# fluggo/Canvas

Hardware: AMD Instinct MI355X
Metric: Mpixels/s through 4K f16 RGBA colour-matrix+alpha-over chain; % HBM roofline (higher is better)
Workload: dtype f32

## Files before the change

### canvas_amd/_lib.py

```python
import ctypes as C
import os

from .abi import (box2i, fir_filter, rational, rgba_frame_f16, rgba_frame_f32, v2f, video_frame_source_funcs,
                  video_source)

_HERE = os.path.dirname(os.path.abspath(__file__))
LIB_PATH = os.path.join(_HERE, "libcanvas_hip.so")

CHAIN_MAX_LAYERS = 8
DISPLAY_RGBA8, DISPLAY_ARGB32_PREMUL = 0, 1
FIR_PATH_AUTO, FIR_PATH_PASSES, FIR_PATH_TILED, FIR_PATH_TABLES, FIR_PATH_HV, FIR_PATH_ONE_COLUMN, FIR_PATH_TWO_COLUMNS, FIR_PATH_STRIPS, FIR_PATH_TILES = 0, 1, 2, 4, 16, 32, 64, 128, 256
FIR_KERNEL_NONE, FIR_KERNEL_WINDOW, FIR_KERNEL_HALVE, _FIR_KERNEL_RETIRED_3, FIR_KERNEL_VH, FIR_KERNEL_TILED, _FIR_KERNEL_RETIRED_6, FIR_KERNEL_TWO_PASS, FIR_KERNEL_PASS, FIR_KERNEL_HV, FIR_KERNEL_WINDOW_PAIR, FIR_KERNEL_HALVE_PAIR, FIR_KERNEL_TILE_VH, FIR_KERNEL_UNSHARP = range(14)
ARITH_SEPARATE, ARITH_CONTRACTED = 0, 1
LUT_NONE, LUT_REC709_TO_LINEAR_SCENE, LUT_REC709_TO_LINEAR_DISPLAY, LUT_LINEAR_TO_REC709, LUT_LINEAR_TO_SRGB = -1, 0, 1, 2, 3
KEY_SHOW_MATTE = 1
MATTE_SHOW, MATTE_MAX_CHOKE, MATTE_MAX_TAPS = 1, 16, 25
TRANSFORM_NEAREST, TRANSFORM_BILINEAR, TRANSFORM_MAX_COORD = 0, 1, 1 << 23
MAX_COORD, RESAMPLE_MAX_COORD = 1 << 30, 1 << 23
YCC_PROGRESSIVE, YCC_REC709 = 1, 2


class rgba_f32(C.Structure):
    _fields_ = [("r", C.c_float), ("g", C.c_float), ("b", C.c_float), ("a", C.c_float)]


class rgba_frame_dev(C.Structure):
    _fields_ = [("data", C.c_void_p), ("format", C.c_int), ("full_window", box2i), ("current_window", box2i),
                ("stream", C.c_void_p)]


class chain_job(C.Structure):
    _fields_ = [("out", C.POINTER(rgba_frame_f16)), ("layers", C.POINTER(rgba_frame_f16) * CHAIN_MAX_LAYERS),
                ("nlayers", C.c_int)]


class chroma_key(C.Structure):
    _fields_ = [("key", C.c_float * 3), ("tolerance", C.c_float), ("softness", C.c_float), ("spill", C.c_float),
                ("spill_range", C.c_float), ("flags", C.c_int)]


class matte_params(C.Structure):
    _fields_ = [("black", C.c_float), ("white", C.c_float), ("choke", C.c_int), ("ntaps", C.c_int), ("taps", C.POINTER(C.c_float)),
                ("flags", C.c_int)]


def matte(choke=0, feather=None, black=0.0, white=1.0, show_matte=False):
    taps = [float(t) for t in feather] if feather is not None else []
    array = (C.c_float * len(taps))(*taps) if taps else None
    m = matte_params(black, white, int(choke), len(taps), C.cast(array, C.POINTER(C.c_float)) if taps else None, MATTE_SHOW if show_matte else 0)
    m._taps = array
    return m


class transform_params(C.Structure):
    _fields_ = [("m", C.c_float * 6), ("filter", C.c_int), ("flags", C.c_int)]


def transform(m=(1.0, 0.0, 0.0, 0.0, 1.0, 0.0), filter=TRANSFORM_BILINEAR):
    return transform_params((C.c_float * 6)(*[float(v) for v in m]), int(filter), 0)


class coded_image(C.Structure):
    _fields_ = [("data", C.c_void_p * 4), ("stride", C.c_int * 4), ("line_count", C.c_int * 4), ("free_func", C.c_void_p)]


P = C.POINTER
rgba_frame_f16_t = rgba_frame_f16
rgba_frame_f32_t = rgba_frame_f32
_u16p, _f32p, _vp = P(C.c_uint16), P(C.c_float), C.c_void_p
_F16, _F32 = P(rgba_frame_f16), P(rgba_frame_f32)

SIGNATURES = {
    "init_half": (None, []),
    "get_frame_time": (C.c_int64, [P(rational), C.c_int]),
    "get_time_frame": (C.c_int, [P(rational), C.c_int64]),
    "gettime": (C.c_int64, []),
    "video_get_frame_f16": (None, [P(video_source), C.c_int, _F16]),
    "video_get_frame_f32": (None, [P(video_source), C.c_int, _F32]),
    "video_get_frame_f16_gl": (None, [P(video_source), C.c_int, _F16]),
    "video_get_frame_f32_gl": (None, [P(video_source), C.c_int, _F32]),
    "video_get_frame_dev": (None, [P(video_source), C.c_int, P(rgba_frame_dev)]),
    "video_copy_frame_f16": (None, [_F16, _F16]),
    "video_copy_frame_alpha_f32": (None, [_F32, _F32, C.c_float]),
    "video_attenuate_f32": (None, [_F32, C.c_float]),
    "cvs_pulldown23_frames": (C.c_int, [C.c_int, C.c_int, P(C.c_int), P(C.c_int)]),
    "cvs_weave_fields_f16_dev": (C.c_int, [_F16, _F16, _vp]),
    "cvs_field_to_frame_f16_dev": (C.c_int, [_F16, _F16, C.c_int, _vp]),
    "cvs_soften_fields_f16_dev": (C.c_int, [_F16, _F16, _vp]),
    "cvs_interlace_fields_f16_dev": (C.c_int, [_F16, _F16, _F16, _vp]),
    "cvs_pulldown23_add_frames": (C.c_int, [C.c_int, C.c_int, P(C.c_int), P(C.c_int)]),
    "video_mix_cross_f32": (None, [_F32, _F32, _F32, C.c_float]),
    "video_mix_cross_f32_pull": (None, [_F32, P(video_source), C.c_int, P(video_source), C.c_int, C.c_float]),
    "video_mix_over_f32": (None, [_F32, _F32, C.c_float]),
    "video_scale_bilinear_f32": (None, [_F32, v2f, _F32, v2f, v2f]),
    "video_scale_bilinear_f32_pull": (None, [_F32, v2f, P(video_source), C.c_int, P(box2i), v2f, v2f]),
    "video_transfer_rec709_to_linear_scene": (None, [_u16p, _u16p, C.c_size_t]),
    "video_transfer_rec709_to_linear_display": (None, [_u16p, _u16p, C.c_size_t]),
    "video_transfer_linear_to_rec709": (None, [_u16p, _u16p, C.c_size_t]),
    "video_transfer_linear_to_sRGB": (None, [_u16p, _u16p, C.c_size_t]),
    "video_get_gamma45_ramp": (P(C.c_uint8), []),
    "video_color_rgb_to_xyz_sdtv": (None, [_F16]),
    "video_color_xyz_to_srgb": (None, [_F16]),
    "filter_createTriangle": (None, [C.c_float, C.c_float, P(fir_filter)]),
    "filter_createLanczos": (None, [C.c_float, C.c_int, C.c_float, P(fir_filter)]),
    "filter_free": (None, [P(fir_filter)]),
    "video_filter_gain_offset_f16": (None, [_F16, _F16, C.c_float, C.c_float]),
    "video_fill_solid_f16": (None, [_F16, P(box2i), P(rgba_f32)]),
    "video_fill_solid_f32": (None, [_F32, P(box2i), P(rgba_f32)]),
    "workspace_create": (_vp, []),
    "workspace_get_length": (C.c_int, [_vp]),
    "workspace_add_item": (_vp, [_vp, _vp, C.c_int64, C.c_int64, C.c_int64, C.c_int64, _vp]),
    "workspace_get_item": (_vp, [_vp, C.c_int]),
    "workspace_remove_item": (None, [_vp]),
    "workspace_as_video_source": (None, [_vp, P(video_source)]),
    "workspace_free": (None, [_vp]),
    "workspace_get_item_pos": (None, [_vp, P(C.c_int64), P(C.c_int64), P(C.c_int64)]),
    "workspace_get_item_offset": (C.c_int64, [_vp]),
    "workspace_set_item_offset": (None, [_vp, C.c_int64]),
    "workspace_get_item_source": (_vp, [_vp]),
    "workspace_set_item_source": (None, [_vp, _vp]),
    "workspace_get_item_tag": (_vp, [_vp]),
    "workspace_set_item_tag": (None, [_vp, _vp]),
    "workspace_update_item": (None, [_vp, P(C.c_int64), P(C.c_int64), P(C.c_int64), P(C.c_int64), P(_vp), P(_vp)]),
    "cvs_set_arithmetic": (C.c_int, [C.c_int]),
    "cvs_get_arithmetic": (C.c_int, []),
    "cvs_init": (C.c_int, [C.c_int]),
    "cvs_device_count": (C.c_int, []),
    "cvs_current_device": (C.c_int, []),
    "cvs_context_open": (C.c_int, [C.c_int]),
    "cvs_context_count": (C.c_int, []),
    "cvs_context_device": (C.c_int, [C.c_int]),
    "cvs_set_context": (C.c_int, [C.c_int]),
    "cvs_current_context": (C.c_int, []),
    "cvs_frame_owner": (C.c_int, [C.c_int64, C.c_int]),
    "cvs_last_error": (C.c_char_p, []),
    "cvs_clear_last_error": (None, []),
    "cvs_set_log_handler": (None, [C.c_void_p, C.c_void_p]),
    "cvs_device_name": (C.c_char_p, []),
    "cvs_compute_units": (C.c_int, []),
    "cvs_malloc": (_vp, [C.c_size_t]),
    "cvs_free": (None, [_vp]),
    "cvs_graph_begin": (C.c_int, [_vp]),
    "cvs_graph_end": (_vp, [_vp]),
    "cvs_graph_launch": (C.c_int, [_vp, _vp]),
    "cvs_graph_destroy": (None, [_vp]),
    "cvs_mem_info": (C.c_int, [P(C.c_size_t), P(C.c_size_t)]),
    "cvs_pool_malloc": (_vp, [C.c_size_t, _vp]),
    "cvs_pool_free": (None, [_vp, _vp]),
    "cvs_pool_trim": (None, []),
    "cvs_thread_release": (None, []),
    "cvs_memcpy_h2d": (C.c_int, [_vp, _vp, C.c_size_t, _vp]),
    "cvs_memcpy_d2h": (C.c_int, [_vp, _vp, C.c_size_t, _vp]),
    "cvs_memcpy_d2d": (C.c_int, [_vp, _vp, C.c_size_t, _vp]),
    "cvs_memset": (C.c_int, [_vp, C.c_int, C.c_size_t, _vp]),
    "cvs_stream_create": (_vp, []),
    "cvs_stream_destroy": (None, [_vp]),
    "cvs_stream_sync": (C.c_int, [_vp]),
    "cvs_event_create": (_vp, []),
    "cvs_event_destroy": (None, [_vp]),
    "cvs_event_record": (C.c_int, [_vp, _vp]),
    "cvs_event_sync": (C.c_int, [_vp]),
    "cvs_event_elapsed_ms": (C.c_float, [_vp, _vp]),
    "cvs_lut_device": (_vp, [C.c_int]),
    "cvs_lut_host": (_u16p, [C.c_int]),
    "cvs_lut_install": (C.c_int, [C.c_int, _u16p]),
    "cvs_half_to_float_dev": (C.c_int, [_vp, _vp, C.c_size_t, _vp]),
    "cvs_float_to_half_dev": (C.c_int, [_vp, _vp, C.c_size_t, _vp]),
    "cvs_half_to_float_fast_dev": (C.c_int, [_vp, _vp, C.c_size_t, _vp]),
    "cvs_float_to_half_fast_dev": (C.c_int, [_vp, _vp, C.c_size_t, _vp]),
    "cvs_half_lookup_dev": (C.c_int, [_vp, _vp, _vp, C.c_size_t, _vp]),
    "cvs_frame_f16_to_f32_dev": (C.c_int, [_F32, _F16, _vp]),
    "cvs_frame_f32_to_f16_dev": (C.c_int, [_F16, _F32, _vp]),
    "cvs_copy_frame_f16_dev": (C.c_int, [_F16, _F16, _vp]),
    "cvs_copy_frame_alpha_f32_dev": (C.c_int, [_F32, _F32, C.c_float, _vp]),
    "cvs_mix_cross_f32_dev": (C.c_int, [_F32, _F32, _F32, C.c_float, _vp]),
    "cvs_mix_over_f32_dev": (C.c_int, [_F32, _F32, C.c_float, _vp]),
    "cvs_color_matrix_f16_dev": (C.c_int, [_F16, _f32p, C.c_int, C.c_int, _vp]),
    "cvs_color_matrix_f16_to_dev": (C.c_int, [_F16, _F16, _f32p, C.c_int, C.c_int, _vp]),
    "cvs_gain_offset_f16_dev": (C.c_int, [_F16, _F16, C.c_float, C.c_float, _vp]),
    "cvs_fill_solid_f16_dev": (C.c_int, [_F16, P(box2i), P(rgba_f32), _vp]),
    "cvs_fill_solid_f32_dev": (C.c_int, [_F32, P(box2i), P(rgba_f32), _vp]),
    "cvs_scale_bilinear_f16_dev": (C.c_int, [_F16, v2f, _F16, v2f, v2f, _vp]),
    "cvs_scale_bilinear_f32_dev": (C.c_int, [_F32, v2f, _F32, v2f, v2f, _vp]),
    "cvs_fir_blur_f32_dev": (C.c_int, [_F32, _F32, _f32p, C.c_int, _vp]),
    "coded_image_alloc": (P(coded_image), [P(C.c_int), P(C.c_int), C.c_int]),
    "coded_image_alloc0": (P(coded_image), [P(C.c_int), P(C.c_int), C.c_int]),
    "video_reconstruct_dv": (None, [_F16, P(coded_image)]),
    "video_subsample_dv": (P(coded_image), [_F16]),
    "cvs_reconstruct_dv_dev": (C.c_int, [_F16, P(coded_image), _vp]),
    "cvs_subsample_dv_dev": (C.c_int, [P(coded_image), _F16, C.c_int, _vp]),
    "video_subsample_mpeg2": (P(coded_image), [_F16]),
    "cvs_subsample_mpeg2_dev": (C.c_int, [P(coded_image), _F16, C.c_int, C.c_int, _vp]),
    "video_reconstruct_mpeg2": (None, [_F16, P(coded_image)]),
    "cvs_reconstruct_mpeg2_dev": (C.c_int, [_F16, P(coded_image), C.c_int, C.c_int, C.c_int, _vp]),
    "cvs_frame_to_bytes_dev": (C.c_int, [_vp, _F16, C.c_int, C.c_int, _vp]),
    "video_frame_to_bytes": (C.c_int, [_vp, _F16, C.c_int, C.c_int]),
    "cvs_frame_to_rgba8_intent_dev": (C.c_int, [_vp, _F16, C.c_int, C.c_float, _vp]),
    "video_frame_to_rgba8_intent": (C.c_int, [_vp, _F16, C.c_int, C.c_float]),
    "cvs_fir_blur_f16_dev": (C.c_int, [_F16, _F16, _f32p, C.c_int, _vp]),
    "cvs_unsharp_mask_f32_dev": (C.c_int, [_F32, _F32, _f32p, C.c_int, C.c_float, C.c_float, _vp]),
    "cvs_unsharp_mask_f16_dev": (C.c_int, [_F16, _F16, _f32p, C.c_int, C.c_float, C.c_float, _vp]),
    "cvs_chroma_key_f32_dev": (C.c_int, [_F32, _F32, P(chroma_key), _vp]),
    "cvs_chroma_key_f16_dev": (C.c_int, [_F16, _F16, P(chroma_key), _vp]),
    "cvs_matte_refine_f32_dev": (C.c_int, [_F32, _F32, P(matte_params), _vp]),
    "cvs_matte_refine_f16_dev": (C.c_int, [_F16, _F16, P(matte_params), _vp]),
    "cvs_transform_f32_dev": (C.c_int, [_F32, _F32, P(transform_params), _vp]),
    "cvs_transform_f16_dev": (C.c_int, [_F16, _F16, P(transform_params), _vp]),
    "cvs_transform_from_parts": (C.c_int, [P(C.c_double), P(C.c_double), C.c_double, P(C.c_double), _f32p]),
    "cvs_transform_target_window": (C.c_int, [P(transform_params), P(box2i), P(box2i), P(box2i)]),
    "cvs_transform_source_window": (C.c_int, [P(transform_params), P(box2i), P(box2i)]),
    "cvs_blur_over_f16_dev": (C.c_int, [_F16, _F16, _f32p, C.c_int, P(_F16), C.c_int, _vp]),
    "cvs_resample_lanczos_f32_dev": (C.c_int, [_F32, _F32, C.c_float, C.c_float, C.c_int, _vp]),
    "cvs_resample_lanczos_f16_dev": (C.c_int, [_F16, _F16, C.c_float, C.c_float, C.c_int, _vp]),
    "cvs_blur_lanczos_f16_dev": (C.c_int, [_F16, _F16, _f32p, C.c_int, C.c_float, C.c_float, C.c_int, _vp]),
    "cvs_blur_over_f16_batch_dev": (C.c_int, [P(_F16), P(_F16), _f32p, C.c_int, P(_F16), C.c_int, C.c_int, _vp]),
    "cvs_scale_bilinear_f16_batch_dev": (C.c_int, [P(_F16), v2f, P(_F16), v2f, v2f, C.c_int, _vp]),
    "cvs_scale_bilinear_f32_batch_dev": (C.c_int, [P(_F32), v2f, P(_F32), v2f, v2f, C.c_int, _vp]),
    "cvs_blur_lanczos_f16_batch_dev": (C.c_int, [P(_F16), P(_F16), C.c_int, _f32p, C.c_int, C.c_float, C.c_float, C.c_int, _vp]),
    "cvs_fir_path_override": (None, [C.c_int]),
    "cvs_chain_color_over_f16_dev": (C.c_int, [P(chain_job), C.c_int, _f32p, C.c_int, C.c_int, _vp]),
    "cvs_chain_last_was_fused": (C.c_int, []),
    "cvs_scale_last_was_fused": (C.c_int, []),
    "cvs_fir_last_kernel": (C.c_int, []),
    "cvs_fir_fell_through_count": (C.c_int, []),
    "cvs_chain_last_launch_count": (C.c_int, []),
    "cvs_mix_cross_f16_dev": (C.c_int, [_F16, _F16, _F16, C.c_float, _vp]),
}

HALF_POINTER_GLOBALS = {
    "half_convert_to_float": C.CFUNCTYPE(None, _f32p, _u16p, C.c_int),
    "half_convert_from_float": C.CFUNCTYPE(None, _u16p, _f32p, C.c_int),
    "half_convert_to_float_fast": C.CFUNCTYPE(None, _f32p, _u16p, C.c_int),
    "half_convert_from_float_fast": C.CFUNCTYPE(None, _u16p, _f32p, C.c_int),
    "half_lookup": C.CFUNCTYPE(None, _u16p, _u16p, _u16p, C.c_int),
}

_lib = None


class LibraryMissing(RuntimeError):
    pass


def load():
    global _lib
    if _lib is not None:
        return _lib
    if not os.path.exists(LIB_PATH):
        raise LibraryMissing(
            "%s not found: build it with `python -c 'import __graft_entry__ as g; g.build()'` "
            "(or make -C canvas_amd/csrc).  There is no CPU fallback." % LIB_PATH)
    lib = C.CDLL(LIB_PATH, mode=C.RTLD_GLOBAL)
    for name, (res, args) in SIGNATURES.items():
        fn = getattr(lib, name)
        fn.restype, fn.argtypes = res, args
    _lib = lib
    return lib


def half_pointer(name):
    lib = load()
    addr = C.c_void_p.in_dll(lib, name).value
    return HALF_POINTER_GLOBALS[name](addr) if addr else None


def last_error():
    return load().cvs_last_error().decode()


def check(rc, what="call"):
    if rc != 0:
        raise RuntimeError("%s failed (%d): %s" % (what, rc, last_error()))
```

### canvas_amd/csrc/host/scale.c

```c
#define _GNU_SOURCE
#include "internal.h"
#include <limits.h>
#include <math.h>
#include <stdatomic.h>

static _Atomic int g_fir_path = CVS_FIR_PATH_AUTO;

static _Thread_local int t_scale_fused;
CVS_EXPORT int cvs_scale_last_was_fused(void) { return t_scale_fused; }
static _Thread_local int t_fir_kernel;
CVS_EXPORT int cvs_fir_last_kernel(void) { return t_fir_kernel; }
static _Thread_local int t_fell_through;
CVS_EXPORT int cvs_fir_fell_through_count(void) { return t_fell_through; }
static void fir_launch_fell_through(const char *kernel, int rc) {
    (void)hipGetLastError();
    t_fell_through++;
    cvs_log_warning("%s did not launch (%s): falling back to the next FIR kernel", kernel, hipGetErrorString((hipError_t)rc));
}
CVS_EXPORT void cvs_fir_path_override(int mode) { atomic_store(&g_fir_path, mode & (CVS_FIR_PATH_PASSES | CVS_FIR_PATH_TILED | CVS_FIR_PATH_TABLES | CVS_FIR_PATH_HV | CVS_FIR_PATH_ONE_COLUMN | CVS_FIR_PATH_TWO_COLUMNS | CVS_FIR_PATH_STRIPS | CVS_FIR_PATH_TILES)); }

typedef struct { void *data; box2i full, cur; int half; } any_frame;

static size_t any_bytes(const any_frame *f) { return cvs_box_pixels(&f->full) * (f->half ? sizeof(rgba_f16) : sizeof(rgba_f32)); }

typedef struct { void *frame, *data; box2i *full, *cur; } frame_ref;

static frame_ref frame_of(const void *f, int half) {
    frame_ref r = { (void *)f, NULL, NULL, NULL };
    if (f && half) { rgba_frame_f16 *h = r.frame; r.data = h->data; r.full = &h->full_window; r.cur = &h->current_window; }
    else if (f)    { rgba_frame_f32 *g = r.frame; r.data = g->data; r.full = &g->full_window; r.cur = &g->current_window; }
    return r;
}

static frame_ref frame_at(const void *frames, int i, int half) {
    return frame_of(half ? (const void *)((const rgba_frame_f16 *const *)frames)[i] : (const void *)((const rgba_frame_f32 *const *)frames)[i], half);
}

static any_frame any_of(const frame_ref *f, int half) {
    const any_frame a = { f->data, *f->full, *f->cur, half };
    return a;
}

static bool entry_refused(void *target, const void *source, int half, const char *what, frame_ref *t, frame_ref *src, int lim) {
    *t = frame_of(target, half);
    *src = frame_of(source, half);
    if (cvs_enter() != 0) { box2i_set_empty(t->cur); return true; }
    if (!cvs_box_contains(src->full, src->cur)) {
        cvs_set_error("%s: the input's current_window lies outside its buffer", what);
        box2i_set_empty(t->cur);
        return true;
    }
    if (cvs_coords_refused(what, "source", src->full, src->cur, lim) || cvs_coords_refused(what, "target", t->full, NULL, lim)) {
        box2i_set_empty(t->cur);
        return true;
    }
    return false;
}

static void batch_empty_from(const void *targets, int from, int count, int half) {
    for (int i = from; i < count; i++) box2i_set_empty(frame_at(targets, i, half).cur);
}

static bool batch_refused(const void *targets, const void *sources, int count, int half, const char *what, int lim) {
    if (!targets || !sources) { cvs_set_error("%s: bad arguments", what); return true; }
    for (int i = 0; i < count; i++)
        if (!frame_at(targets, i, half).frame || !frame_at(sources, i, half).frame) {
            cvs_set_error("%s: frame %d of %d is a null pointer", what, i, count);
            return true;
        }
    for (int i = 0; i < count; i++) {
        const frame_ref src = frame_at(sources, i, half);
        if (!cvs_box_contains(src.full, src.cur)) {
            cvs_set_error("%s: the input's current_window lies outside its buffer (frame %d)", what, i);
            batch_empty_from(targets, 0, count, half);
            return true;
        }
        if (cvs_coords_refused(what, "a source", src.full, src.cur, lim) || cvs_coords_refused(what, "a target", frame_at(targets, i, half).full, NULL, lim)) {
            batch_empty_from(targets, 0, count, half);
            return true;
        }
    }
    if (cvs_enter() != 0) { batch_empty_from(targets, 0, count, half); return true; }
    return false;
}

static bool same_box(const box2i *a, const box2i *b) { return memcmp(a, b, sizeof *a) == 0; }

static bool batch_group(cvk_frame_batch *b, const void *targets, const void *sources, int half, int first, int n, size_t tbytes, size_t sbytes,
                        const rgba_frame_f16 *const *overlays, int noverlays) {
    const void *in[CVK_FRAME_BATCH * (1 + CVK_BLUR_MAX_OVER)];
    int nin = 0;
    memset(b, 0, sizeof *b);
    b->n = n;
    for (int i = 0; i < n; i++) {
        b->target[i] = frame_at(targets, first + i, half).data;
        in[nin++] = b->source[i] = frame_at(sources, first + i, half).data;
        for (int l = 0; l < noverlays; l++) in[nin++] = b->over[i][l] = overlays[(size_t)(first + i) * noverlays + l]->data;
    }
    if (n < 2) return false;
    for (int i = 0; i < n; i++) {
        const char *o = b->target[i];
        for (int j = 0; j < nin; j++) { const char *q = in[j]; if (q && o < q + sbytes && q < o + tbytes) return false; }
        for (int j = 0; j < i; j++) { const char *q = b->target[j]; if (o < q + tbytes && q < o + tbytes) return false; }
    }
    return true;
}

static int gather_pass(const any_frame *t, const any_frame *src, const cvk_fir_axis *tab, int axis, int t0, int t1, int lo, int hi, hipStream_t s) {
    if (t1 < t0 || hi < lo) return 0;
    cvk_fir_params fp;
    memset(&fp, 0, sizeof fp);
    fp.target = cvs_view(t->data, &t->full);
    fp.source = cvs_view(src->data, &src->full);
    fp.axis = axis;
    fp.t0 = t0; fp.t1 = t1; fp.lo = lo; fp.hi = hi;
    fp.ntaps = tab->ntaps; fp.tap_src = tab->src; fp.taps = tab->taps; fp.stride = tab->stride;
    fp.in_half = src->half; fp.out_half = t->half;
    return CVK(cvk_fir_gather)(&fp, s);
}

static cvk_fir2d_params fir2d_params(const any_frame *t, const any_frame *src, int tx0, int ty0, int tx1, int ty1,
                                     const cvs_fir_table *h, const cvs_fir_table *v) {
    cvk_fir2d_params fp;
    memset(&fp, 0, sizeof fp);
    fp.target = cvs_view(t->data, &t->full);
    fp.source = cvs_view(src->data, &src->full);
    fp.in_half = src->half; fp.out_half = t->half;
    fp.tx0 = tx0; fp.ty0 = ty0; fp.tx1 = tx1; fp.ty1 = ty1;
    fp.h = h->axis; fp.v = v->axis;
    fp.max_sw = h->max_foot > 0 ? h->max_foot : 1;
    return fp;
}


static int triangle_pass(any_frame *target, float tmin, const any_frame *source, float smin, float factor, int axis, hipStream_t s) {
    const box2i srect = source->cur, trect = target->full;
    const int lo = axis ? (srect.min.y > trect.min.y ? srect.min.y : trect.min.y) : (srect.min.x > trect.min.x ? srect.min.x : trect.min.x);
    const int hi = axis ? (srect.max.y < trect.max.y ? srect.max.y : trect.max.y) : (srect.max.x < trect.max.x ? srect.max.x : trect.max.x);
    const int s0 = axis ? srect.min.x : srect.min.y, s1 = axis ? srect.max.x : srect.max.y;
    const int t0 = axis ? trect.min.x : trect.min.y, t1 = axis ? trect.max.x : trect.max.y;

    cvs_fir_table table;
    int rc = cvs_fir_table_triangle(tmin, smin, factor, s0, s1, t0, t1, axis == 0 || lo <= hi, &table);
    if (rc != 0) return rc;
    const int used_lo = table.used_lo, used_hi = table.used_hi;
    {
        const int o0 = axis ? trect.min.y : trect.min.x, o1 = axis ? trect.max.y : trect.max.x;
        const bool covers = used_hi >= used_lo && hi >= lo && used_lo == t0 && used_hi == t1 && lo == o0 && hi == o1;
        if (!covers && any_bytes(target)) {
            hipError_t e_ = hipMemsetAsync(target->data, 0, any_bytes(target), s);
            if (e_ != hipSuccess) { cvs_fir_table_release(&table, s); cvs_set_error("zero fill: %s", hipGetErrorString(e_)); return -1; }
        }
    }
    if (used_hi >= used_lo && hi >= lo) {
        const size_t first = (size_t)(used_lo - t0);
        cvk_fir_axis from = table.axis;
        from.ntaps += first; from.src += first * (size_t)from.stride; from.taps += first * (size_t)from.stride;
        rc = gather_pass(target, source, &from, axis, used_lo, used_hi, lo, hi, s);
        if (rc == 0) t_fir_kernel = CVS_FIR_KERNEL_PASS;
    }
    cvs_fir_table_release(&table, s);
    if (rc != 0) { cvs_set_error("FIR gather launch failed: %s", hipGetErrorString((hipError_t)rc)); return rc; }
    if (axis) box2i_set(&target->cur, used_lo, lo, used_hi, hi);
    else      box2i_set(&target->cur, lo, used_lo, hi, used_hi);
    return 0;
}

static int triangle_fused_vh(any_frame *target, v2f tp, const any_frame *source, v2f sp, v2f fac, const box2i *mid_full,
                             const cvk_frame_batch *batch, hipStream_t s) {
    const box2i *tf = &target->full, *sc = &source->cur;
    const int lo1 = sc->min.x > mid_full->min.x ? sc->min.x : mid_full->min.x, hi1 = sc->max.x < mid_full->max.x ? sc->max.x : mid_full->max.x;
    cvs_fir_table tv, th = { .pin = -1 };
    if (hi1 < lo1) return 1;
    if (cvs_fir_table_triangle(tp.y, sp.y, fac.y, sc->min.y, sc->max.y, mid_full->min.y, mid_full->max.y, true, &tv) != 0) return -1;
    const int vlo = tv.used_lo, vhi = tv.used_hi;
    int rc = 1;
    if (vhi >= vlo) {
        const int lo2 = vlo > tf->min.y ? vlo : tf->min.y, hi2 = vhi < tf->max.y ? vhi : tf->max.y;
        if (hi2 >= lo2 && cvs_fir_table_triangle(tp.x, sp.x, fac.x, lo1, hi1, tf->min.x, tf->max.x, true, &th) == 0) {
            const int hlo = th.used_lo, hhi = th.used_hi;
            cvk_fir2d_params fp = fir2d_params(target, source, tf->min.x, mid_full->min.y, tf->max.x, hi2, &th, &tv);
            const int pinned = atomic_load(&g_fir_path);
            const bool tiles = hhi >= hlo && !(pinned & CVS_FIR_PATH_STRIPS) &&
                               ((pinned & CVS_FIR_PATH_TILES) ? CVK(cvk_fir_tvh_supported)(&fp)
                                : batch && target->half ? false : CVK(cvk_fir_tvh_preferred)(&fp));
            bool alike = true;
            for (int i = 0; batch && i < batch->n; i++) alike = alike && !((((uintptr_t)batch->target[i]) ^ (uintptr_t)target->data) & 15u);
            if (batch && !(alike && hhi >= hlo && (tiles || CVK(cvk_fir_vh_supported)(&fp)))) rc = 2;
            else if (hhi >= hlo && (tiles || CVK(cvk_fir_vh_supported)(&fp))) {
                const bool covers = lo2 == tf->min.y && hi2 == tf->max.y;
                hipError_t e = hipSuccess;
                if (batch) {
                    fp.nframes = batch->n;
                    for (int i = 0; i < batch->n; i++) {
                        fp.frame_source[i] = batch->source[i]; fp.frame_target[i] = batch->target[i];
                        if (!covers && any_bytes(target) && e == hipSuccess) e = hipMemsetAsync(batch->target[i], 0, any_bytes(target), s);
                    }
                } else if (!covers && any_bytes(target)) e = hipMemsetAsync(target->data, 0, any_bytes(target), s);
                int krc = e != hipSuccess ? (int)e : tiles ? CVK(cvk_fir_tvh)(&fp, lo2 - fp.ty0, s) : CVK(cvk_fir_vh)(&fp, lo2 - fp.ty0, cvs_cus(), s);
                if (krc == 0) { box2i_set(&target->cur, hlo, lo2, hhi, hi2); t_fir_kernel = tiles ? CVS_FIR_KERNEL_TILE_VH : CVS_FIR_KERNEL_VH; rc = 0; }
                else { fir_launch_fell_through(tiles ? "k_fir_tile_vh" : "k_fir_vh", krc); rc = 1; }
            }
        }
    }
    cvs_fir_table_release(&tv, s); cvs_fir_table_release(&th, s);
    return rc;
}

static int triangle_fused_hv(any_frame *target, v2f tp, const any_frame *source, v2f sp, v2f fac, const box2i *mid_full, hipStream_t s) {
    const box2i *tf = &target->full, *sc = &source->cur;
    const int lo1 = sc->min.y > mid_full->min.y ? sc->min.y : mid_full->min.y, hi1 = sc->max.y < mid_full->max.y ? sc->max.y : mid_full->max.y;
    cvs_fir_table th, tv = { .pin = -1 };
    if (hi1 < lo1) return 1;
    if (cvs_arith() != CVS_ARITH_SEPARATE) return 1;
    if (cvs_fir_table_triangle(tp.x, sp.x, fac.x, sc->min.x, sc->max.x, mid_full->min.x, mid_full->max.x, true, &th) != 0) return -1;
    const int hlo = th.used_lo, hhi = th.used_hi;
    int rc = 1;
    if (hhi >= hlo) {
        const int lo2 = hlo > tf->min.x ? hlo : tf->min.x, hi2 = hhi < tf->max.x ? hhi : tf->max.x;
        if (hi2 >= lo2 && cvs_fir_table_triangle(tp.y, sp.y, fac.y, lo1, hi1, tf->min.y, tf->max.y, true, &tv) == 0) {
            const int vlo = tv.used_lo, vhi = tv.used_hi;
            cvk_fir2d_params fp = fir2d_params(target, source, mid_full->min.x, tf->min.y, hi2, tf->max.y, &th, &tv);
            if (vhi >= vlo && cvk_fir_hv_supported(&fp)) {
                const bool covers = fp.tx0 == tf->min.x && hi2 == tf->max.x;
                hipError_t e = covers || !any_bytes(target) ? hipSuccess : hipMemsetAsync(target->data, 0, any_bytes(target), s);
                int krc = e != hipSuccess ? (int)e : cvk_fir_hv(&fp, cvs_cus(), s);
                if (krc == 0) { box2i_set(&target->cur, lo2, vlo, hi2, vhi); t_fir_kernel = CVS_FIR_KERNEL_HV; rc = 0; }
                else { fir_launch_fell_through("k_fir_hv", krc); rc = 1; }
            }
        }
    }
    cvs_fir_table_release(&tv, s); cvs_fir_table_release(&th, s);
    return rc;
}

static int scale_core(any_frame *target, v2f tp, const any_frame *source, v2f sp, v2f fac, const cvk_frame_batch *batch, hipStream_t s) {
    t_scale_fused = 0;
    t_fir_kernel = CVS_FIR_KERNEL_NONE;
    if (batch && ((fac.x == 1.0f && tp.x == sp.x) || (fac.y == 1.0f && tp.y == sp.y) || fac.x < fac.y ||
                  (atomic_load(&g_fir_path) & (CVS_FIR_PATH_PASSES | CVS_FIR_PATH_TILED)))) return 2;
    if (fac.x == 1.0f && tp.x == sp.x) return triangle_pass(target, tp.y, source, sp.y, fac.y, 0, s);
    if (fac.y == 1.0f && tp.y == sp.y) return triangle_pass(target, tp.x, source, sp.x, fac.x, 1, s);

    any_frame mid;
    memset(&mid, 0, sizeof mid);
    const box2i *tf = &target->full, *sc = &source->cur;
    const bool x_first = fac.x < fac.y;
    const int fl = cvs_arith() == CVS_ARITH_CONTRACTED;
    if (x_first)
        box2i_set(&mid.full, (int)madd_as(fl, -(tp.x - tf->min.x), fac.x, sp.x), sc->min.y,
                  (int)madd_as(fl, tf->max.x - tp.x, fac.x, sp.x), sc->max.y);
    else
        box2i_set(&mid.full, sc->min.x, (int)madd_as(fl, -(tp.y - tf->min.y), fac.y, sp.y),
                  sc->max.x, (int)madd_as(fl, tf->max.y - tp.y, fac.y, sp.y));
    box2i_intersect(&mid.full, &mid.full, tf);
    mid.cur = mid.full;
    if (!(atomic_load(&g_fir_path) & (CVS_FIR_PATH_PASSES | CVS_FIR_PATH_TILED))) {
        int rc = x_first ? triangle_fused_hv(target, tp, source, sp, fac, &mid.full, s) : triangle_fused_vh(target, tp, source, sp, fac, &mid.full, batch, s);
        if (rc == 0) t_scale_fused = 1;
        if (rc <= 0) return rc;
        if (batch) return 2;
    }
    size_t n = cvs_box_pixels(&mid.full);
    mid.data = cvs_pool_malloc(sizeof(rgba_f32) * (n ? n : 1), s);
    if (!mid.data) return -1;
    int rc;
    if (x_first) { rc = triangle_pass(&mid, tp.x, source, sp.x, fac.x, 1, s); if (rc == 0) rc = triangle_pass(target, tp.y, &mid, sp.y, fac.y, 0, s); }
    else         { rc = triangle_pass(&mid, tp.y, source, sp.y, fac.y, 0, s); if (rc == 0) rc = triangle_pass(target, tp.x, &mid, sp.x, fac.x, 1, s); }
    cvs_pool_free(mid.data, s);
    return rc;
}

static int scale_frame(void *target, v2f tp, const void *source, v2f sp, v2f fac, int half, cvs_stream_t stream, const char *what) {
    frame_ref t, src;
    if (entry_refused(target, source, half, what, &t, &src, CVS_RESAMPLE_MAX_COORD)) return -1;
    if (cvs_point_refused(what, "the target point", tp, CVS_RESAMPLE_MAX_COORD) || cvs_point_refused(what, "the source point", sp, CVS_RESAMPLE_MAX_COORD)) {
        box2i_set_empty(t.cur);
        return -1;
    }
    hipStream_t s = cvs_pick_stream(stream);
    if (fac.x == 1.0f && tp.x == sp.x && fac.y == 1.0f && tp.y == sp.y)
        return half ? cvs_copy_frame_f16_dev(target, source, s) : cvs_copy_frame_alpha_f32_dev(target, source, 1.0f, s);
    any_frame tf = any_of(&t, half);
    const any_frame sf = any_of(&src, half);
    int rc = scale_core(&tf, tp, &sf, sp, fac, NULL, s);
    *t.cur = tf.cur;
    if (rc != 0) box2i_set_empty(t.cur);
    return rc;
}

CVS_EXPORT int cvs_scale_bilinear_f32_dev(rgba_frame_f32 *target, v2f tp, const rgba_frame_f32 *source, v2f sp, v2f fac, cvs_stream_t stream) {
    return scale_frame(target, tp, source, sp, fac, 0, stream, "cvs_scale_bilinear_f32_dev");
}

CVS_EXPORT int cvs_scale_bilinear_f16_dev(rgba_frame_f16 *target, v2f tp, const rgba_frame_f16 *source, v2f sp, v2f fac, cvs_stream_t stream) {
    return scale_frame(target, tp, source, sp, fac, 1, stream, "cvs_scale_bilinear_f16_dev");
}

static int scale_batch_frames(const void *targets, v2f tp, const void *sources, v2f sp, v2f fac, int count, int half,
                              cvs_stream_t stream, const char *what) {
    if (count <= 0) return 0;
    if (batch_refused(targets, sources, count, half, what, CVS_RESAMPLE_MAX_COORD)) return -1;
    if (cvs_point_refused(what, "the target point", tp, CVS_RESAMPLE_MAX_COORD) || cvs_point_refused(what, "the source point", sp, CVS_RESAMPLE_MAX_COORD)) {
        batch_empty_from(targets, 0, count, half);
        return -1;
    }
    hipStream_t s = cvs_pick_stream(stream);
    const size_t px = half ? sizeof(rgba_f16) : sizeof(rgba_f32);
    int rc = 0, done = 0;
    for (int base = 0; count > 1 && rc == 0 && done == base && base < count; base += 64) {
        const int end = count - base < 64 ? count : base + 64;
        const frame_ref t0 = frame_at(targets, base, half), s0 = frame_at(sources, base, half);
        bool uniform = end - base > 1 && !box2i_is_empty(s0.cur) && !box2i_is_empty(t0.full) &&
                       !(fac.x == 1.0f && tp.x == sp.x && fac.y == 1.0f && tp.y == sp.y);
        for (int i = base + 1; uniform && i < end; i++) {
            const frame_ref ti = frame_at(targets, i, half), si = frame_at(sources, i, half);
            uniform = same_box(ti.full, t0.full) && same_box(si.full, s0.full) && same_box(si.cur, s0.cur);
        }
        const size_t tbytes = cvs_box_pixels(t0.full) * px, sbytes = cvs_box_pixels(s0.full) * px;
        while (uniform && rc == 0 && done < end) {
            const int n = end - done < CVK_FRAME_BATCH ? end - done : CVK_FRAME_BATCH;
            cvk_frame_batch b;
            if (!batch_group(&b, targets, sources, half, done, n, tbytes, sbytes, NULL, 0)) break;
            const frame_ref td = frame_at(targets, done, half), sd = frame_at(sources, done, half);
            any_frame t = any_of(&td, half);
            const any_frame src = any_of(&sd, half);
            rc = scale_core(&t, tp, &src, sp, fac, &b, s);
            if (rc == 2) { rc = 0; break; }
            if (rc != 0) break;
            for (int i = 0; i < n; i++) *frame_at(targets, done + i, half).cur = t.cur;
            done += n;
        }
    }
    for (; rc == 0 && done < count; done++) {
        void *t = frame_at(targets, done, half).frame;
        const void *src = frame_at(sources, done, half).frame;
        rc = half ? cvs_scale_bilinear_f16_dev(t, tp, src, sp, fac, stream) : cvs_scale_bilinear_f32_dev(t, tp, src, sp, fac, stream);
    }
    if (rc != 0) batch_empty_from(targets, done, count, half);
    return rc;
}

CVS_EXPORT int cvs_scale_bilinear_f16_batch_dev(rgba_frame_f16 *const *targets, v2f tp, const rgba_frame_f16 *const *sources, v2f sp, v2f fac, int count, cvs_stream_t stream) {
    return scale_batch_frames(targets, tp, sources, sp, fac, count, 1, stream, "cvs_scale_bilinear_f16_batch_dev");
}

CVS_EXPORT int cvs_scale_bilinear_f32_batch_dev(rgba_frame_f32 *const *targets, v2f tp, const rgba_frame_f32 *const *sources, v2f sp, v2f fac, int count, cvs_stream_t stream) {
    return scale_batch_frames(targets, tp, sources, sp, fac, count, 0, stream, "cvs_scale_bilinear_f32_batch_dev");
}

CVS_EXPORT void video_scale_bilinear_f32(rgba_frame_f32 *target, v2f tp, rgba_frame_f32 *source, v2f sp, v2f fac) {
    cvs_bridge br;
    rgba_frame_f32 ft, fs;
    cvs_bridge_open(&br);
    CVS_BRIDGE_FRAME(&br, ft, target, CVS_BRIDGE_UPLOAD);
    CVS_BRIDGE_FRAME(&br, fs, source, CVS_BRIDGE_PRIVATE | (box2i_is_empty(&source->current_window) ? 0 : CVS_BRIDGE_UPLOAD));
    CVS_BRIDGE_CALL(&br, cvs_scale_bilinear_f32_dev, &ft, tp, &fs, sp, fac);
    target->current_window = ft.current_window;
    if (cvs_bridge_close(&br, target->data) != 0) box2i_set_empty(&target->current_window);
}

CVS_EXPORT void video_scale_bilinear_f32_pull(rgba_frame_f32 *target, v2f tp, video_source *source, int frame,
                                              box2i *source_rect, v2f sp, v2f fac) {
    if (fac.x == 0.0f || fac.y == 0.0f) { box2i_set_empty(&target->current_window); return; }
    if (fac.x == 1.0f && fac.y == 1.0f && tp.x == sp.x && tp.y == sp.y) { video_get_frame_f32(source, frame, target); return; }
    const box2i *tf = &target->full_window;
    if (cvs_coords_refused("video_scale_bilinear_f32_pull", "target", tf, NULL, CVS_RESAMPLE_MAX_COORD) ||
        cvs_point_refused("video_scale_bilinear_f32_pull", "the target point", tp, CVS_RESAMPLE_MAX_COORD) ||
        cvs_point_refused("video_scale_bilinear_f32_pull", "the source point", sp, CVS_RESAMPLE_MAX_COORD)) {
        box2i_set_empty(&target->current_window);
        return;
    }
    rgba_frame_f32 tmp;
    box2i_set(&tmp.full_window,
              (int)(sp.x - (tp.x - tf->min.x) / fac.x) - 1, (int)(sp.y - (tp.y - tf->min.y) / fac.y) - 1,
              (int)(sp.x + (tf->max.x - tp.x) / fac.x) + 1, (int)(sp.y + (tf->max.y - tp.y) / fac.y) + 1);
    box2i_intersect(&tmp.full_window, &tmp.full_window, source_rect);
    tmp.current_window = tmp.full_window;
    size_t n = cvs_box_pixels(&tmp.full_window);
    tmp.data = malloc(sizeof(rgba_f32) * (n ? n : 1));
    if (!tmp.data) { box2i_set_empty(&target->current_window); return; }
    video_get_frame_f32(source, frame, &tmp);
    video_scale_bilinear_f32(target, tp, &tmp, sp, fac);
    free(tmp.data);
}


static int fir_two_launches(const any_frame *t, const any_frame *src, const box2i *rect, const cvk_fir_axis *h, const cvk_fir_axis *v, hipStream_t s) {
    const box2i *sw = &src->cur;
    any_frame mid = { NULL, *sw, *sw, 0 };
    box2i_set(&mid.full, rect->min.x, sw->min.y, rect->max.x, sw->max.y);
    mid.data = cvs_pool_malloc(cvs_box_pixels(&mid.full) * sizeof(rgba_f32), s);
    if (!mid.data) return -1;
    int rc = gather_pass(&mid, src, h, 1, rect->min.x, rect->max.x, sw->min.y, sw->max.y, s);
    if (rc == 0) rc = gather_pass(t, &mid, v, 0, rect->min.y, rect->max.y, rect->min.x, rect->max.x, s);
    cvs_pool_free(mid.data, s);
    if (rc != 0) { cvs_set_error("FIR gather launch failed: %s", hipGetErrorString((hipError_t)rc)); return -1; }
    t_fir_kernel = CVS_FIR_KERNEL_TWO_PASS;
    return 0;
}

static int fir2d_launch(const any_frame *t, const any_frame *src, const box2i *rect, const cvs_fir_table *h, const cvs_fir_table *v, hipStream_t s) {
    cvk_fir2d_params fp = fir2d_params(t, src, rect->min.x, rect->min.y, rect->max.x, rect->max.y, h, v);
    fp.max_sh = v->max_foot > 0 ? v->max_foot : 1;
    const int force = atomic_load(&g_fir_path);
    if (force & CVS_FIR_PATH_PASSES) return 1;
    const bool pinned = (force & (CVS_FIR_PATH_TILED | CVS_FIR_PATH_HV)) != 0;
    if (cvs_arith() == CVS_ARITH_SEPARATE && ((force & CVS_FIR_PATH_HV) || !pinned) && cvk_fir_hv_supported(&fp)) {
        int rc = cvk_fir_hv(&fp, cvs_cus(), s);
        if (rc == 0) { t_fir_kernel = CVS_FIR_KERNEL_HV; return 0; }
        fir_launch_fell_through("k_fir_hv", rc);
    }
    if (CVK(cvk_fir2d_lds_bytes)(&fp) > 150 * 1024 || h->axis.stride > 64 || v->axis.stride > 64) return 1;
    int rc = CVK(cvk_fir2d)(&fp, s);
    if (rc != 0) { cvs_set_error("fused FIR launch failed: %s", hipGetErrorString((hipError_t)rc)); return -1; }
    t_fir_kernel = CVS_FIR_KERNEL_TILED;
    return 0;
}

static int fir_pair_launch(const any_frame *t, const any_frame *src, const box2i *rect, cvs_fir_table *h, cvs_fir_table *v, hipStream_t s) {
    int rc = fir2d_launch(t, src, rect, h, v, s);
    if (rc == 1) rc = fir_two_launches(t, src, rect, &h->axis, &v->axis, s);
    cvs_fir_table_release(h, s); cvs_fir_table_release(v, s);
    return rc;
}

static int blur_column_pins(void) {
    const int pin = atomic_load(&g_fir_path);
    return (pin & CVS_FIR_PATH_ONE_COLUMN ? CVK_BLUR_ONE_COLUMN : 0) | (pin & CVS_FIR_PATH_TWO_COLUMNS ? CVK_BLUR_TWO_COLUMNS : 0);
}

static bool blur_has_fast_kernel(const float *taps, int ntaps) {
    bool finite = true;
    for (int k = 0; k < ntaps; k++) finite = finite && isfinite(taps[k]);
    return finite && CVK(cvk_blur_supported)(ntaps, 1) && !(atomic_load(&g_fir_path) & CVS_FIR_PATH_TABLES);
}

static bool halving_sweep(cvk_blur_halve_params *hp, float fx, float fy, int ksize, const float *taps, int ntaps, const any_frame *t, const any_frame *src) {
    if (fx != 0.5f || fy != 0.5f || (atomic_load(&g_fir_path) & CVS_FIR_PATH_TABLES)) return false;
    const box2i *tf = &t->full, *sw = &src->cur;
    fir_filter f = { NULL, 0, 0 };
    filter_createLanczos(0.5f, ksize, 0.0f, &f);
    bool usable = f.coeff && f.center == f.width / 2 && f.width <= 16 && ntaps <= 16 &&
                  tf->min.x > -(1 << 22) && tf->max.x < (1 << 22) && tf->min.y > -(1 << 22) && tf->max.y < (1 << 22);
    for (int k = 0; usable && k < f.width; k++) usable = isfinite(f.coeff[k]);
    for (int k = 0; usable && k < ntaps; k++) usable = isfinite(taps[k]);
    if (usable) {
        memset(hp, 0, sizeof *hp);
        hp->target = cvs_view(t->data, tf);
        hp->source = cvs_view(src->data, &src->full);
        hp->in_half = 1; hp->out_half = 1;
        hp->tx0 = tf->min.x; hp->ty0 = tf->min.y; hp->tx1 = tf->max.x; hp->ty1 = tf->max.y;
        hp->sx0 = sw->min.x; hp->sy0 = sw->min.y; hp->sx1 = sw->max.x; hp->sy1 = sw->max.y;
        hp->ntaps1 = ntaps; hp->ntaps2 = f.width;
        memcpy(hp->taps1, taps, sizeof(float) * (size_t)ntaps);
        memcpy(hp->taps2, f.coeff, sizeof(float) * (size_t)f.width);
        hp->flags = blur_column_pins();
    }
    filter_free(&f);
    return usable;
}

static int halving_launch(const cvk_blur_halve_params *hp, hipStream_t s) {
    int rc = CVK(cvk_blur_halve)(hp, cvs_cus(), s);
    if (rc != 0) { cvs_set_error("blur + halving launch failed: %s", hipGetErrorString((hipError_t)rc)); return -1; }
    t_fir_kernel = CVK(cvk_blur_halve_takes_pairs)(hp) ? CVS_FIR_KERNEL_HALVE_PAIR : CVS_FIR_KERNEL_HALVE;
    return 0;
}

static int blur_fused(const any_frame *t, const any_frame *src, const box2i *win, const float *taps, int ntaps,
                      const void *const *over, int nover, const cvk_frame_batch *batch, hipStream_t s) {
    const box2i *sw = &src->cur;
    if (blur_has_fast_kernel(taps, ntaps)) {
        cvk_blur_params bp;
        memset(&bp, 0, sizeof bp);
        bp.nover = nover;
        for (int l = 0; l < nover; l++) bp.over[l] = over[l];
        bp.target = cvs_view(t->data, &t->full);
        bp.source = cvs_view(src->data, &src->full);
        bp.in_half = src->half; bp.out_half = t->half;
        bp.tx0 = win->min.x; bp.ty0 = win->min.y; bp.tx1 = win->max.x; bp.ty1 = win->max.y;
        bp.sx0 = sw->min.x; bp.sy0 = sw->min.y; bp.sx1 = sw->max.x; bp.sy1 = sw->max.y;
        bp.ntaps = ntaps;
        memcpy(bp.taps, taps, sizeof(float) * (size_t)ntaps);
        if (batch) {
            if (!(ntaps & 1) || ntaps > 31) return 1;
            bp.batch = *batch;
        }
        bp.flags = blur_column_pins();
        int rc = CVK(cvk_blur)(&bp, cvs_cus(), s);
        if (rc != 0) { cvs_set_error("blur launch failed: %s", hipGetErrorString((hipError_t)rc)); return -1; }
        t_fir_kernel = CVK(cvk_blur_takes_pairs)(&bp) ? CVS_FIR_KERNEL_WINDOW_PAIR : CVS_FIR_KERNEL_WINDOW;
        return 0;
    }
    if (nover > 0 || batch) return 1;
    cvs_fir_table h, v;
    if (cvs_fir_table_blur(taps, ntaps, win->min.x, win->max.x, sw->min.x, sw->max.x, CVK_FIR2D_TILE_X, &h) != 0) return -1;
    if (cvs_fir_table_blur(taps, ntaps, win->min.y, win->max.y, sw->min.y, sw->max.y, CVK_FIR2D_TILE_Y, &v) != 0) { cvs_fir_table_release(&h, s); return -1; }
    return fir_pair_launch(t, src, win, &h, &v, s);
}

static int lanczos_fused(const any_frame *t, const any_frame *src, float fx, float fy, int ksize, hipStream_t s) {
    const box2i *tfull = &t->full, *sw = &src->cur;
    const float identity = 1.0f;
    cvk_blur_halve_params hp;
    if (halving_sweep(&hp, fx, fy, ksize, &identity, 1, t, src) && CVK(cvk_blur_supported)(hp.ntaps2, 2)) {
        int rc, kernel;
        if (src->half && t->half && CVK(cvk_blur_halve_takes_pairs)(&hp)) {
            rc = CVK(cvk_blur_halve_pair)(&hp, cvs_cus(), s);
            kernel = CVS_FIR_KERNEL_HALVE_PAIR;
        } else {
            cvk_blur_params bp;
            memset(&bp, 0, sizeof bp);
            bp.target = hp.target; bp.source = hp.source;
            bp.in_half = src->half; bp.out_half = t->half;
            bp.tx0 = hp.tx0; bp.ty0 = hp.ty0; bp.tx1 = hp.tx1; bp.ty1 = hp.ty1;
            bp.sx0 = hp.sx0; bp.sy0 = hp.sy0; bp.sx1 = hp.sx1; bp.sy1 = hp.sy1;
            bp.ntaps = hp.ntaps2; bp.step = 2;
            memcpy(bp.taps, hp.taps2, sizeof(float) * (size_t)hp.ntaps2);
            rc = CVK(cvk_blur)(&bp, cvs_cus(), s);
            kernel = CVS_FIR_KERNEL_WINDOW;
        }
        if (rc != 0) { cvs_set_error("resample launch failed: %s", hipGetErrorString((hipError_t)rc)); return -1; }
        t_fir_kernel = kernel;
        return 0;
    }
    cvs_fir_table h, v;
    if (cvs_fir_table_lanczos(fx, ksize, tfull->min.x, tfull->max.x, sw->min.x, sw->max.x, CVK_FIR2D_TILE_X, &h) != 0) return -1;
    if (cvs_fir_table_lanczos(fy, ksize, tfull->min.y, tfull->max.y, sw->min.y, sw->max.y, CVK_FIR2D_TILE_Y, &v) != 0) { cvs_fir_table_release(&h, s); return -1; }
    return fir_pair_launch(t, src, tfull, &h, &v, s);
}

static int fir_blur(void *target, const void *source, const float *taps, int ntaps, int half, cvs_stream_t stream, const char *what) {
    frame_ref t, src;
    if (entry_refused(target, source, half, what, &t, &src, CVS_MAX_COORD)) return -1;
    if (ntaps < 1 || !taps) { cvs_set_error("blur: need at least one tap"); box2i_set_empty(t.cur); return -1; }
    hipStream_t s = cvs_pick_stream(stream);
    box2i win;
    box2i_intersect(&win, src.cur, t.full);
    *t.cur = win;
    if (box2i_is_empty(&win)) return 0;
    const any_frame tf = any_of(&t, half), sf = any_of(&src, half);
    int rc = blur_fused(&tf, &sf, &win, taps, ntaps, NULL, 0, NULL, s);
    if (rc != 0) box2i_set_empty(t.cur);
    return rc;
}

CVS_EXPORT int cvs_fir_blur_f32_dev(rgba_frame_f32 *target, const rgba_frame_f32 *source, const float *taps, int ntaps, cvs_stream_t stream) {
    return fir_blur(target, source, taps, ntaps, 0, stream, "cvs_fir_blur_f32_dev");
}

CVS_EXPORT int cvs_fir_blur_f16_dev(rgba_frame_f16 *target, const rgba_frame_f16 *source, const float *taps, int ntaps, cvs_stream_t stream) {
    return fir_blur(target, source, taps, ntaps, 1, stream, "cvs_fir_blur_f16_dev");
}

static int unsharp_mask(void *target, const void *source, const float *taps, int ntaps, float amount, float threshold, int half,
                        cvs_stream_t stream, const char *what) {
    frame_ref t, src;
    if (entry_refused(target, source, half, what, &t, &src, CVS_MAX_COORD)) return -1;
    if (ntaps < 1 || !taps) { cvs_set_error("unsharp mask: need at least one tap"); box2i_set_empty(t.cur); return -1; }
    hipStream_t s = cvs_pick_stream(stream);
    box2i win;
    box2i_intersect(&win, src.cur, t.full);
    *t.cur = win;
    const bool fused = blur_has_fast_kernel(taps, ntaps) && CVK(cvk_unsharp_supported)(ntaps);
    t_fir_kernel = fused ? CVS_FIR_KERNEL_UNSHARP : CVS_FIR_KERNEL_NONE;
    if (box2i_is_empty(&win)) return 0;
    const any_frame tf = any_of(&t, half), sf = any_of(&src, half);
    int rc;
    if (fused) {
        cvk_unsharp_params up;
        memset(&up, 0, sizeof up);
        up.target = cvs_view(tf.data, &tf.full);
        up.source = cvs_view(sf.data, &sf.full);
        up.half = half;
        up.tx0 = win.min.x; up.ty0 = win.min.y; up.tx1 = win.max.x; up.ty1 = win.max.y;
        up.sx0 = sf.cur.min.x; up.sy0 = sf.cur.min.y; up.sx1 = sf.cur.max.x; up.sy1 = sf.cur.max.y;
        up.ntaps = ntaps;
        up.amount = amount; up.threshold = threshold;
        memcpy(up.taps, taps, sizeof(float) * (size_t)ntaps);
        rc = CVK(cvk_unsharp)(&up, cvs_cus(), s);
        if (rc != 0) { cvs_set_error("unsharp mask launch failed: %s", hipGetErrorString((hipError_t)rc)); rc = -1; }
    } else {
        any_frame mid = { NULL, win, win, 0 };
        mid.data = cvs_pool_malloc(cvs_box_pixels(&win) * sizeof(rgba_f32), s);
        if (!mid.data) { box2i_set_empty(t.cur); return -1; }
        rc = blur_fused(&mid, &sf, &win, taps, ntaps, NULL, 0, NULL, s);
        if (rc == 0) {
            const cvk_rect r = { win.min.x, win.min.y, win.max.x, win.max.y };
            rc = CVK(cvk_unsharp_combine)(cvs_view(tf.data, &tf.full), cvs_view(sf.data, &sf.full), cvs_view(mid.data, &mid.full), r, half, amount, threshold, s);
            if (rc != 0) { cvs_set_error("unsharp mask launch failed: %s", hipGetErrorString((hipError_t)rc)); rc = -1; }
        }
        cvs_pool_free(mid.data, s);
    }
    if (rc != 0) box2i_set_empty(t.cur);
    return rc;
}

CVS_EXPORT int cvs_unsharp_mask_f32_dev(rgba_frame_f32 *target, const rgba_frame_f32 *source, const float *taps, int ntaps, float amount, float threshold, cvs_stream_t s) {
    return unsharp_mask(target, source, taps, ntaps, amount, threshold, 0, s, "cvs_unsharp_mask_f32_dev");
}

CVS_EXPORT int cvs_unsharp_mask_f16_dev(rgba_frame_f16 *target, const rgba_frame_f16 *source, const float *taps, int ntaps, float amount, float threshold, cvs_stream_t s) {
    return unsharp_mask(target, source, taps, ntaps, amount, threshold, 1, s, "cvs_unsharp_mask_f16_dev");
}

CVS_EXPORT int cvs_blur_over_f16_dev(rgba_frame_f16 *out, const rgba_frame_f16 *source, const float *taps, int ntaps,
                                     const rgba_frame_f16 *const *overlays, int noverlays, cvs_stream_t stream) {
    if (cvs_enter() != 0) { box2i_set_empty(&out->current_window); return -1; }
    CVS_REQUIRE_INSIDE(source, out, "cvs_blur_over_f16_dev");
    CVS_REQUIRE_COORDS(source, 1, out, "cvs_blur_over_f16_dev", "source");
    CVS_REQUIRE_COORDS(out, 0, out, "cvs_blur_over_f16_dev", "out");
    for (int l = 0; l < noverlays && overlays; l++) CVS_REQUIRE_COORDS(overlays[l], 1, out, "cvs_blur_over_f16_dev", "an overlay");
    if (ntaps < 1 || !taps || noverlays < 0 || (noverlays > 0 && !overlays)) { cvs_set_error("blur+over: bad arguments"); box2i_set_empty(&out->current_window); return -1; }
    if (noverlays == 0) return cvs_fir_blur_f16_dev(out, source, taps, ntaps, stream);
    hipStream_t s = cvs_pick_stream(stream);
    const box2i *full = &out->full_window;
    if (box2i_is_empty(full)) { box2i_set_empty(&out->current_window); return 0; }
    const any_frame o = { out->data, *full, *full, 1 }, src = { (void *)source->data, source->full_window, source->current_window, 1 };
    box2i win;
    box2i_intersect(&win, &source->current_window, full);
    bool whole = noverlays <= CVK_BLUR_MAX_OVER && memcmp(&win, full, sizeof win) == 0;
    const void *bufs[CVK_BLUR_MAX_OVER];
    for (int l = 0; whole && l < noverlays; l++) {
        whole = memcmp(&overlays[l]->full_window, full, sizeof *full) == 0 && memcmp(&overlays[l]->current_window, full, sizeof *full) == 0;
        bufs[l] = overlays[l]->data;
    }
    int rc = 1;
    if (whole && noverlays > 0) rc = blur_fused(&o, &src, &win, taps, ntaps, bufs, noverlays, NULL, s);
    if (rc == 0) { out->current_window = *full; return 0; }
    if (rc < 0) { box2i_set_empty(&out->current_window); return rc; }

    rgba_frame_f32 acc = { cvs_pool_malloc(cvs_box_pixels(full) * sizeof(rgba_f32), s), *full, *full };
    rgba_frame_f32 tmp = { noverlays > 0 ? cvs_pool_malloc(cvs_box_pixels(full) * sizeof(rgba_f32), s) : NULL, *full, *full };
    rc = (acc.data && (tmp.data || noverlays == 0)) ? 0 : -1;
    if (rc == 0) {
        box2i_set_empty(&acc.current_window);
        if (!box2i_is_empty(&win)) {
            const any_frame a = { acc.data, *full, win, 0 };
            acc.current_window = win;
            rc = blur_fused(&a, &src, &win, taps, ntaps, NULL, 0, NULL, s);
        }
    }
    for (int l = 0; rc == 0 && l < noverlays; l++) {
        rc = cvs_frame_f16_to_f32_dev(&tmp, overlays[l], s);
        if (rc == 0) rc = cvs_mix_over_f32_dev(&acc, &tmp, 1.0f, s);
    }
    if (rc == 0) rc = cvs_frame_f32_to_f16_dev(out, &acc, s);
    cvs_pool_free(acc.data, s); cvs_pool_free(tmp.data, s);
    if (rc != 0) box2i_set_empty(&out->current_window);
    return rc;
}

static int resample_lanczos(void *target, const void *source, float fx, float fy, int ksize, int half, cvs_stream_t stream, const char *what) {
    frame_ref t, src;
    if (entry_refused(target, source, half, what, &t, &src, CVS_RESAMPLE_MAX_COORD)) return -1;
    if (!(fx > 0.0f) || !(fy > 0.0f) || ksize < 1 || box2i_is_empty(src.cur) || box2i_is_empty(t.full)) {
        box2i_set_empty(t.cur);
        return 0;
    }
    hipStream_t s = cvs_pick_stream(stream);
    const any_frame tf = any_of(&t, half), sf = any_of(&src, half);
    int rc = lanczos_fused(&tf, &sf, fx, fy, ksize, s);
    if (rc == 0) *t.cur = *t.full;
    else box2i_set_empty(t.cur);
    return rc;
}

CVS_EXPORT int cvs_resample_lanczos_f32_dev(rgba_frame_f32 *target, const rgba_frame_f32 *source, float fx, float fy, int ksize, cvs_stream_t stream) {
    return resample_lanczos(target, source, fx, fy, ksize, 0, stream, "cvs_resample_lanczos_f32_dev");
}

CVS_EXPORT int cvs_resample_lanczos_f16_dev(rgba_frame_f16 *target, const rgba_frame_f16 *source, float fx, float fy, int ksize, cvs_stream_t stream) {
    return resample_lanczos(target, source, fx, fy, ksize, 1, stream, "cvs_resample_lanczos_f16_dev");
}

CVS_EXPORT int cvs_blur_lanczos_f16_dev(rgba_frame_f16 *target, const rgba_frame_f16 *source, const float *taps, int ntaps,
                                        float fx, float fy, int ksize, cvs_stream_t stream) {
    if (cvs_enter() != 0) { box2i_set_empty(&target->current_window); return -1; }
    CVS_REQUIRE_INSIDE(source, target, "cvs_blur_lanczos_f16_dev");
    if (cvs_coords_refused("cvs_blur_lanczos_f16_dev", "source", &source->full_window, &source->current_window, CVS_RESAMPLE_MAX_COORD) ||
        cvs_coords_refused("cvs_blur_lanczos_f16_dev", "target", &target->full_window, NULL, CVS_RESAMPLE_MAX_COORD)) {
        box2i_set_empty(&target->current_window);
        return -1;
    }
    if (ntaps < 1 || !taps || !(fx > 0.0f) || !(fy > 0.0f) || ksize < 1) { cvs_set_error("blur+lanczos: bad arguments"); box2i_set_empty(&target->current_window); return -1; }
    if (box2i_is_empty(&source->current_window) || box2i_is_empty(&target->full_window)) { box2i_set_empty(&target->current_window); return 0; }
    hipStream_t s = cvs_pick_stream(stream);
    const box2i *sw = &source->current_window;
    const any_frame tf = { target->data, target->full_window, target->full_window, 1 }, sf = { (void *)source->data, source->full_window, *sw, 1 };
    if (ntaps == 1 && taps[0] == 1.0f) return cvs_resample_lanczos_f16_dev(target, source, fx, fy, ksize, stream);
    cvk_blur_halve_params hp;
    if ((ntaps & 1) && halving_sweep(&hp, fx, fy, ksize, taps, ntaps, &tf, &sf) && CVK(cvk_blur_halve_supported)(ntaps, hp.ntaps2)) {
        const int rc = halving_launch(&hp, s);
        if (rc == 0) target->current_window = target->full_window;
        else box2i_set_empty(&target->current_window);
        return rc;
    }
    any_frame mid = { NULL, *sw, *sw, 0 };
    mid.data = cvs_pool_malloc(cvs_box_pixels(sw) * sizeof(rgba_f32), s);
    if (!mid.data) { box2i_set_empty(&target->current_window); return -1; }
    int rc = blur_fused(&mid, &sf, sw, taps, ntaps, NULL, 0, NULL, s);
    if (rc == 0) rc = lanczos_fused(&tf, &mid, fx, fy, ksize, s);
    if (rc == 0) target->current_window = target->full_window;
    cvs_pool_free(mid.data, s);
    if (rc != 0) box2i_set_empty(&target->current_window);
    return rc;
}

CVS_EXPORT int cvs_blur_over_f16_batch_dev(rgba_frame_f16 *const *outs, const rgba_frame_f16 *const *sources, const float *taps, int ntaps,
                                           const rgba_frame_f16 *const *overlays, int noverlays, int count, cvs_stream_t stream) {
    const char *what = "cvs_blur_over_f16_batch_dev";
    if (count <= 0) return 0;
    if (ntaps < 1 || !taps || noverlays < 0 || (noverlays > 0 && !overlays)) { cvs_set_error("%s: bad arguments", what); return -1; }
    for (int i = 0; i < count; i++)
        for (int l = 0; l < noverlays; l++)
            if (!overlays[(size_t)i * noverlays + l]) { cvs_set_error("%s: layer %d of frame %d is a null pointer", what, l, i); return -1; }
    if (batch_refused(outs, sources, count, 1, what, CVS_MAX_COORD)) return -1;
    for (int i = 0; i < count * noverlays; i++)
        if (cvs_coords_refused(what, "an overlay", &overlays[i]->full_window, &overlays[i]->current_window, CVS_MAX_COORD)) { batch_empty_from(outs, 0, count, 1); return -1; }
    hipStream_t s = cvs_pick_stream(stream);
    const box2i *full = &outs[0]->full_window;
    bool uniform = count > 1 && noverlays >= 1 && noverlays <= CVK_BLUR_MAX_OVER && !box2i_is_empty(full) && blur_has_fast_kernel(taps, ntaps) && (ntaps & 1);
    for (int i = 0; uniform && i < count; i++) {
        uniform = same_box(&outs[i]->full_window, full) && same_box(&sources[i]->full_window, &sources[0]->full_window) &&
                  same_box(&sources[i]->current_window, full) && same_box(&sources[0]->full_window, full);
        for (int l = 0; uniform && l < noverlays; l++) {
            const rgba_frame_f16 *ov = overlays[(size_t)i * noverlays + l];
            uniform = same_box(&ov->full_window, full) && same_box(&ov->current_window, full);
        }
    }
    int rc = 0, done = 0;
    const size_t bytes = cvs_box_pixels(full) * sizeof(rgba_f16);
    while (uniform && rc == 0 && done < count) {
        const int n = count - done < CVK_FRAME_BATCH ? count - done : CVK_FRAME_BATCH;
        cvk_frame_batch b;
        if (!batch_group(&b, outs, sources, 1, done, n, bytes, bytes, overlays, noverlays)) break;
        const any_frame t = { b.target[0], *full, *full, 1 }, src = { (void *)b.source[0], sources[done]->full_window, sources[done]->current_window, 1 };
        rc = blur_fused(&t, &src, full, taps, ntaps, b.over[0], noverlays, &b, s);
        if (rc == 1) { rc = 0; break; }
        if (rc == 0) { for (int i = 0; i < n; i++) outs[done + i]->current_window = *full; done += n; }
    }
    for (; rc == 0 && done < count; done++)
        rc = cvs_blur_over_f16_dev(outs[done], sources[done], taps, ntaps, noverlays ? overlays + (size_t)done * noverlays : NULL, noverlays, stream);
    if (rc != 0) batch_empty_from(outs, done, count, 1);
    return rc;
}

CVS_EXPORT int cvs_blur_lanczos_f16_batch_dev(rgba_frame_f16 *const *targets, const rgba_frame_f16 *const *sources, int count,
                                              const float *taps, int ntaps, float fx, float fy, int ksize, cvs_stream_t stream) {
    const char *what = "cvs_blur_lanczos_f16_batch_dev";
    if (count <= 0) return 0;
    if (ntaps < 1 || !taps || !(fx > 0.0f) || !(fy > 0.0f) || ksize < 1) { cvs_set_error("%s: bad arguments", what); return -1; }
    if (batch_refused(targets, sources, count, 1, what, CVS_RESAMPLE_MAX_COORD)) return -1;
    hipStream_t s = cvs_pick_stream(stream);
    int rc = 0, done = 0;
    const box2i *tf = &targets[0]->full_window, *sw = &sources[0]->current_window;
    bool uniform = count > 1 && (ntaps & 1) && !(ntaps == 1 && taps[0] == 1.0f) && !box2i_is_empty(sw) && !box2i_is_empty(tf);
    for (int i = 1; uniform && i < count; i++)
        uniform = same_box(&targets[i]->full_window, tf) && same_box(&sources[i]->full_window, &sources[0]->full_window) &&
                  same_box(&sources[i]->current_window, sw);
    const any_frame t0 = { targets[0]->data, *tf, *tf, 1 }, s0 = { (void *)sources[0]->data, sources[0]->full_window, *sw, 1 };
    cvk_blur_halve_params hp;
    if (uniform && halving_sweep(&hp, fx, fy, ksize, taps, ntaps, &t0, &s0) && CVK(cvk_blur_halve_supported)(ntaps, hp.ntaps2)) {
        const size_t sbytes = cvs_box_pixels(&sources[0]->full_window) * sizeof(rgba_f16), tbytes = cvs_box_pixels(tf) * sizeof(rgba_f16);
        while (rc == 0 && done < count) {
            const int n = count - done < CVK_FRAME_BATCH ? count - done : CVK_FRAME_BATCH;
            if (!batch_group(&hp.batch, targets, sources, 1, done, n, tbytes, sbytes, NULL, 0)) break;
            hp.target.data = hp.batch.target[0];
            hp.source.data = (void *)hp.batch.source[0];
            if ((rc = halving_launch(&hp, s)) != 0) break;
            for (int i = 0; i < n; i++) targets[done + i]->current_window = targets[done + i]->full_window;
            done += n;
        }
    }
    for (; rc == 0 && done < count; done++)
        rc = cvs_blur_lanczos_f16_dev(targets[done], sources[done], taps, ntaps, fx, fy, ksize, stream);
    if (rc != 0) batch_empty_from(targets, done, count, 1);
    return rc;
}
```

### canvas_amd/csrc/kernels/chain_kernel.hpp

```cpp
#pragma once
#include "lut_common.hpp"
#include "grade.hpp"
#include "chain_math.hpp"
#include <string.h>

namespace {

using namespace cvs;

template <int ML> struct JobCT { void *out; const void *layer[ML]; uint64_t npixels; };
template <int ML> struct BatchT {
    static constexpr int kJobs = ML == 4 ? 64 : 48;
    JobCT<ML> jobs[kJobs];
};
template <int ML>
inline int fill_batch(BatchT<ML> &b, const cvk_chain_job *jobs, int njobs, int nlayers, uint64_t bytes_per_launch) {
    memset(&b, 0, sizeof b);
    uint64_t bytes = 0;
    int n = 0;
    while (n < njobs && n < BatchT<ML>::kJobs) {
        const cvk_chain_job &src = jobs[n];
        const uint64_t job_bytes = src.npixels * 8 * (uint64_t)(nlayers + 1);
        if (n > 0 && bytes + job_bytes > bytes_per_launch) break;
        b.jobs[n].out = src.out;
        for (int k = 0; k < nlayers; k++) b.jobs[n].layer[k] = src.layer[k];
        b.jobs[n].npixels = src.npixels;
        bytes += job_bytes;
        n++;
    }
    return n;
}
static_assert(sizeof(BatchT<4>) + 160 <= 4096 && sizeof(BatchT<8>) + 160 <= 4096, "kernel arguments must fit the 4 KiB segment");

template <int MAXL, bool PRE, bool POST>
__device__ __forceinline__ uint2 chain_pixel(const uint2 (&px)[MAXL], int nl, const MatR &mat, const uint16_t *lut, const uint16_t *post) {
    if (MAXL >= 2 && mat.cross) return narrow(blend_cross(widen(px[0]), widen(px[MAXL >= 2 ? 1 : 0]), mat.wa, mat.wb));
    px32 acc = mat.plain ? widen(px[0]) : grade<PRE, POST>(px[0], mat, lut, post);
#pragma unroll
    for (int k = 1; k < MAXL; k++)
        if (k < nl) acc = blend_over(acc, mat.plain ? widen(px[k]) : grade<PRE, POST>(px[k], mat, lut, post), 1.0f);
    return narrow(acc);
}


__device__ __forceinline__ void asm_ld4s(u32x4 &dst, const void *sbase, uint32_t voff) {
    asm volatile("global_load_dwordx4 %0, %1, %2 nt" : "=v"(dst) : "v"(voff), "s"(sbase));
}

template <int L>
__device__ __forceinline__ void wait_vm0(u32x4 (&r)[L]) {
    static_assert(L >= 1 && L <= 8, "operand lists below cover 1..8 layers");
    if constexpr (L == 1) asm volatile("s_waitcnt vmcnt(0)" : "+v"(r[0]) : : "memory");
    else if constexpr (L == 2) asm volatile("s_waitcnt vmcnt(0)" : "+v"(r[0]), "+v"(r[1]) : : "memory");
    else if constexpr (L == 3) asm volatile("s_waitcnt vmcnt(0)" : "+v"(r[0]), "+v"(r[1]), "+v"(r[2]) : : "memory");
    else if constexpr (L == 4) asm volatile("s_waitcnt vmcnt(0)" : "+v"(r[0]), "+v"(r[1]), "+v"(r[2]), "+v"(r[3]) : : "memory");
    else if constexpr (L == 5) asm volatile("s_waitcnt vmcnt(0)" : "+v"(r[0]), "+v"(r[1]), "+v"(r[2]), "+v"(r[3]), "+v"(r[4]) : : "memory");
    else if constexpr (L == 6) asm volatile("s_waitcnt vmcnt(0)" : "+v"(r[0]), "+v"(r[1]), "+v"(r[2]), "+v"(r[3]), "+v"(r[4]), "+v"(r[5]) : : "memory");
    else if constexpr (L == 7) asm volatile("s_waitcnt vmcnt(0)" : "+v"(r[0]), "+v"(r[1]), "+v"(r[2]), "+v"(r[3]), "+v"(r[4]), "+v"(r[5]), "+v"(r[6]) : : "memory");
    else asm volatile("s_waitcnt vmcnt(0)" : "+v"(r[0]), "+v"(r[1]), "+v"(r[2]), "+v"(r[3]), "+v"(r[4]), "+v"(r[5]), "+v"(r[6]), "+v"(r[7]) : : "memory");
}

__device__ __forceinline__ void stage_lut_any(uint16_t *lds, const uint16_t *__restrict__ table) {
    const uint4 *src = reinterpret_cast<const uint4 *>(table);
    uint4 *dst = reinterpret_cast<uint4 *>(lds);
    constexpr int kWords = kLutHalfs * 2 / 16;
    if (kWords % blockDim.x == 0) {
        const int slices = kWords / (int)blockDim.x, rot = (int)(blockIdx.x >> 3);
        for (int it = 0; it < slices; it++) {
            const int i = ((it + rot) % slices) * (int)blockDim.x + (int)threadIdx.x;
            dst[i] = src[i];
        }
    } else {
        for (int i = threadIdx.x; i < kWords; i += blockDim.x) dst[i] = src[i];
    }
    __syncthreads();
}

enum { DIAG_NONE = 0, DIAG_MEMORY_ONLY = 1, DIAG_COMPUTE_ONLY = 2 };

template <int NL>
struct Walk {
    unsigned job;
    unsigned chunk;
    unsigned npairs;
    unsigned nchunks;
    const char *layer[NL];
    char *out;
};

constexpr bool chain_hand_pipelined(int nl, int mode, bool pre, bool post) {
    return !(nl == 6 && mode == CHAIN_GRADE && pre && !post);
}

template <int NL, int MODE, bool PRE, bool POST, int DIAG>
__global__ __launch_bounds__(NL <= 4 ? kWG : 512) void k_chain(BatchT<(NL <= 4 ? 4 : 8)> batch, int njobs_, Mat kmat, int lshift,
                                               const uint16_t *__restrict__ pre, const uint16_t *__restrict__ post) {
    constexpr bool HAND = chain_hand_pipelined(NL, MODE, PRE, POST);
    const MatR mat = CVS_MAT_REGS(kmat);
    __shared__ uint16_t lut[(PRE || POST) ? kLutHalfs : 1];
    const unsigned L = 1u << lshift, G = gridDim.x, tid = threadIdx.x, njobs = (unsigned)njobs_;

    auto load_job = [&](Walk<NL> &w) {
        const auto &job = batch.jobs[w.job];
        w.npairs = (unsigned)(job.npixels >> 1);
        w.nchunks = (w.npairs + L - 1) >> lshift;
#pragma unroll
        for (int k = 0; k < NL; k++) w.layer[k] = reinterpret_cast<const char *>(job.layer[k]);
        w.out = reinterpret_cast<char *>(job.out);
    };
    auto advance = [&](Walk<NL> &w, unsigned by) {
        w.chunk += by;
        while (w.chunk >= w.nchunks) {
            w.chunk -= w.nchunks;
            if (++w.job >= njobs) { w.job = njobs; w.chunk = 0; return; }
            load_job(w);
        }
    };
    auto valid_of = [&](const Walk<NL> &w) -> unsigned { const unsigned left = w.npairs - (w.chunk << lshift); return left < L ? left : L; };
    auto issue = [&](u32x4 (&dst)[NL], const Walk<NL> &w) {
        const unsigned valid = valid_of(w);
        const uint32_t voff = (tid < valid ? tid : valid - 1) << 4;
#pragma unroll
        for (int k = 0; k < NL; k++) {
            const char *base = w.layer[k] + ((size_t)w.chunk << (lshift + 4));
            if constexpr (HAND) asm_ld4s(dst[k], base, voff);
            else dst[k] = __builtin_nontemporal_load(reinterpret_cast<const u32x4 *>(base + voff));
        }
    };

    Walk<NL> cur;
    cur.job = 0; cur.chunk = 0;
    load_job(cur);
    advance(cur, blockIdx.x);
    if (cur.job >= njobs) return;
    Walk<NL> next = cur;
    advance(next, G);

    u32x4 A[NL], B[NL];
    u32x4 diag_acc = { 0, 0, 0, 0 };
    issue(A, cur);
    if (PRE) stage_lut_any(lut, pre);
    else if (POST) stage_lut_any(lut, post);
    if constexpr (HAND) wait_vm0(A);
    if (next.job < njobs) issue(B, next);

    auto trip = [&](u32x4 (&now)[NL], u32x4 (&nxt)[NL]) -> bool {
        u32x4 res;
        if (DIAG == DIAG_MEMORY_ONLY) {
            res = now[0];
#pragma unroll
            for (int k = 1; k < NL; k++) res ^= now[k];
        } else {
            res = chain_pair_lean<NL, PRE, POST, MODE>(now, mat, lut, post);
        }
        Walk<NL> after = next;
        if (after.job < njobs) advance(after, G);
        const bool store_it = tid < valid_of(cur);
        g_u4 out = (g_u4)(cur.out + ((size_t)cur.chunk << (lshift + 4)));
        __builtin_amdgcn_sched_barrier(0);
        if constexpr (HAND) wait_vm0(nxt);
        __builtin_amdgcn_sched_barrier(0);
        if (DIAG == DIAG_COMPUTE_ONLY) diag_acc ^= res;
        else if (store_it) __builtin_nontemporal_store(res, out + tid);
        if (after.job < njobs) {
            if (DIAG == DIAG_COMPUTE_ONLY) {
#pragma unroll
                for (int k = 0; k < NL; k++) now[k] = nxt[k];
            } else {
                issue(now, after);
            }
        }
        __builtin_amdgcn_sched_barrier(0);
        cur = next;
        next = after;
        return cur.job < njobs;
    };
    while (trip(A, B) && trip(B, A)) { }
    if (DIAG == DIAG_COMPUTE_ONLY) ((g_u4)batch.jobs[0].out)[(size_t)blockIdx.x * L + tid] = diag_acc;

}

template <int NL, int MODE, bool PRE, bool POST>
__global__ __launch_bounds__(64) void k_chain_tail(BatchT<(NL <= 4 ? 4 : 8)> batch, int njobs, Mat kmat, const uint16_t *__restrict__ pre, const uint16_t *__restrict__ post) {
    MatR mat = CVS_MAT_REGS(kmat);
    mat.plain = MODE == CHAIN_PLAIN; mat.cross = MODE == CHAIN_CROSS;
    const int j = (int)threadIdx.x;
    if (j >= njobs) return;
    const auto &job = batch.jobs[j];
    if (!(job.npixels & 1)) return;
    uint2 px[NL];
#pragma unroll
    for (int k = 0; k < NL; k++) px[k] = ld2(job.layer[k], job.npixels - 1);
    st2(job.out, job.npixels - 1, chain_pixel<NL, PRE, POST>(px, NL, mat, PRE ? pre : post, post));
}

template <int NL, int MODE, int DIAG>
int launch(const BatchT<(NL <= 4 ? 4 : 8)> &jobs, int njobs, const Mat &mat, const uint16_t *pre, const uint16_t *post, unsigned grid, unsigned block, int lshift, hipStream_t s) {
    bool odd = false;
    for (int i = 0; i < njobs; i++) odd = odd || (jobs.jobs[i].npixels & 1);
    if constexpr (MODE != CHAIN_GRADE) {
        hipLaunchKernelGGL((k_chain<NL, MODE, false, false, DIAG>), dim3(grid), dim3(block), 0, s, jobs, njobs, mat, lshift, pre, post);
        if (odd) hipLaunchKernelGGL((k_chain_tail<NL, MODE, false, false>), dim3(1), dim3(64), 0, s, jobs, njobs, mat, pre, post);
    } else {
        if (pre && post)  hipLaunchKernelGGL((k_chain<NL, MODE, true, true, DIAG>), dim3(grid), dim3(block), 0, s, jobs, njobs, mat, lshift, pre, post);
        else if (pre)     hipLaunchKernelGGL((k_chain<NL, MODE, true, false, DIAG>), dim3(grid), dim3(block), 0, s, jobs, njobs, mat, lshift, pre, post);
        else if (post)    hipLaunchKernelGGL((k_chain<NL, MODE, false, true, DIAG>), dim3(grid), dim3(block), 0, s, jobs, njobs, mat, lshift, pre, post);
        else              hipLaunchKernelGGL((k_chain<NL, MODE, false, false, DIAG>), dim3(grid), dim3(block), 0, s, jobs, njobs, mat, lshift, pre, post);
        if (odd) {
            if (pre && post)  hipLaunchKernelGGL((k_chain_tail<NL, MODE, true, true>), dim3(1), dim3(64), 0, s, jobs, njobs, mat, pre, post);
            else if (pre)     hipLaunchKernelGGL((k_chain_tail<NL, MODE, true, false>), dim3(1), dim3(64), 0, s, jobs, njobs, mat, pre, post);
            else if (post)    hipLaunchKernelGGL((k_chain_tail<NL, MODE, false, true>), dim3(1), dim3(64), 0, s, jobs, njobs, mat, pre, post);
            else              hipLaunchKernelGGL((k_chain_tail<NL, MODE, false, false>), dim3(1), dim3(64), 0, s, jobs, njobs, mat, pre, post);
        }
    }
    return (int)hipGetLastError();
}


}
```

### canvas_amd/csrc/kernels/kernels.h

```cpp
#ifndef CVS_KERNELS_H
#define CVS_KERNELS_H

#include <stddef.h>
#include <stdint.h>

#ifdef CVS_DIAG
#include <stdlib.h>
#define CVS_DIAG_ENV(name) getenv(name)
#else
#define CVS_DIAG_ENV(name) ((const char *)0)
#endif

#ifdef CVS_CONTRACT
#define cvk_gain_offset_f16          cvk_gain_offset_f16_fma
#define cvk_mix                      cvk_mix_fma
#define cvk_color_matrix             cvk_color_matrix_fma
#define cvk_chain_color_over         cvk_chain_color_over_fma
#define cvk_chain_cross              cvk_chain_cross_fma
#define cvk_chain_count_reset        cvk_chain_count_reset_fma
#define cvk_chain_count              cvk_chain_count_fma
#define cvk_fir_gather               cvk_fir_gather_fma
#define cvk_fir2d_lds_bytes          cvk_fir2d_lds_bytes_fma
#define cvk_fir2d                    cvk_fir2d_fma
#define cvk_fir_vh_supported         cvk_fir_vh_supported_fma
#define cvk_fir_vh                   cvk_fir_vh_fma
#define cvk_fir_tvh_supported        cvk_fir_tvh_supported_fma
#define cvk_fir_tvh_preferred        cvk_fir_tvh_preferred_fma
#define cvk_fir_tvh                  cvk_fir_tvh_fma
#define cvk_blur_supported           cvk_blur_supported_fma
#define cvk_blur_takes_pairs         cvk_blur_takes_pairs_fma
#define cvk_blur                     cvk_blur_fma
#define cvk_blur_pair_supported      cvk_blur_pair_supported_fma
#define cvk_blur_pair                cvk_blur_pair_fma
#define cvk_blur_halve_pair_supported cvk_blur_halve_pair_supported_fma
#define cvk_blur_halve_pair          cvk_blur_halve_pair_fma
#define cvk_blur_halve_supported     cvk_blur_halve_supported_fma
#define cvk_blur_halve_takes_pairs   cvk_blur_halve_takes_pairs_fma
#define cvk_blur_halve               cvk_blur_halve_fma
#define cvk_unsharp_supported        cvk_unsharp_supported_fma
#define cvk_unsharp                  cvk_unsharp_fma
#define cvk_unsharp_combine          cvk_unsharp_combine_fma
#define cvk_dv_reconstruct           cvk_dv_reconstruct_fma
#define cvk_dv_subsample             cvk_dv_subsample_fma
#endif

#ifdef __cplusplus
extern "C" {
#endif

typedef struct {
    void *data;
    int pitch;
    int fx0, fy0, fx1, fy1;
} cvk_view;

typedef struct { int x0, y0, x1, y1; } cvk_rect;

int cvk_half_to_float(float *out, const uint16_t *in, size_t count, int fast, void *stream);
int cvk_float_to_half(uint16_t *out, const float *in, size_t count, int fast, void *stream);
int cvk_half_lookup(const uint16_t *table, uint16_t *out, const uint16_t *in, size_t count, int cus, void *stream);

int cvk_copy_f16(cvk_view out, cvk_view in, cvk_rect r, void *stream);
int cvk_copy_alpha_f32(cvk_view out, cvk_view in, cvk_rect r, float alpha, void *stream);
int cvk_weave_f16(cvk_view frame, cvk_rect cur, const void *other, cvk_rect other_cur, void *stream);
int cvk_widen(cvk_view out32, cvk_view in16, cvk_rect r, void *stream);
int cvk_narrow(cvk_view out16, cvk_view in32, cvk_rect r, void *stream);
int cvk_fill_f16(cvk_view out, cvk_rect r, const float rgba[4], void *stream);
int cvk_fill_f32(cvk_view out, cvk_rect r, const float rgba[4], void *stream);
int cvk_gain_offset_f16(cvk_view out, cvk_view in, cvk_rect r, float gain, float offset, void *stream);

enum { CVK_MIX_CROSS = 0, CVK_MIX_OVER = 1 };
typedef struct {
    cvk_view out, p, q;
    cvk_rect outer, inner;
    cvk_rect pw, qw;
    int gap_x, gap_y;
    int top_is_p, bottom_is_p, left_is_p, right_is_p;
    float wp, wq;
    int mode;
    int p_in_place;
} cvk_mix_params;
int cvk_mix(const cvk_mix_params *mp, void *stream);

int cvk_color_matrix(cvk_view dst, cvk_view src, cvk_rect r, const float m[9], const uint16_t *pre_lut,
                     const uint16_t *post_lut, int cus, void *stream);

#define CVK_CHAIN_MAX_LAYERS 8
typedef struct {
    void *out;
    const void *layer[CVK_CHAIN_MAX_LAYERS];
    int nlayers;
    int pad;
    uint64_t npixels;
} cvk_chain_job;
int cvk_chain_color_over(const cvk_chain_job *jobs, int njobs, int uniform_layers, const float *m,
                         const uint16_t *pre_lut, const uint16_t *post_lut, int cus, void *stream);

void cvk_chain_count_reset(void);
int cvk_chain_count(void);

int cvk_chain_cross(const cvk_chain_job *jobs, int njobs, float wa, float wb, int cus, void *stream);

typedef struct {
    cvk_view target, source;
    int axis;
    int t0, t1;
    int lo, hi;
    int s0, s1;
    const int *ntaps;
    const int *tap_src;
    const float *taps;
    int stride;
    int in_half, out_half;
} cvk_fir_params;
int cvk_fir_gather(const cvk_fir_params *fp, void *stream);
int cvk_zero_f32(cvk_view v, void *stream);

typedef struct {
    const int *ntaps, *src;
    const float *taps;
    const int *foot;
    int stride;
    int lines;
    int max_taps;
    int wide_foot;
    int max_active;
    int streamable;
    const uint32_t *lrec;
    const uint32_t *pack;
    int pack_width;
    int span_lines[3];
} cvk_fir_axis;
#define CVK_FIR_LREC 32
#define CVK_AXIS_ALIGN(bytes)              (((size_t)(bytes) + 255) & ~(size_t)255)
#define CVK_AXIS_NLINES(lines)             ((size_t)((lines) > 0 ? (lines) : 1))
#define CVK_AXIS_OFF_SRC(lines)            CVK_AXIS_ALIGN(CVK_AXIS_NLINES(lines) * 4)
#define CVK_AXIS_OFF_TAPS(lines, stride)   (CVK_AXIS_OFF_SRC(lines) + CVK_AXIS_ALIGN(CVK_AXIS_NLINES(lines) * (size_t)(stride) * 4))
#define CVK_AXIS_OFF_FOOT(lines, stride)   (CVK_AXIS_OFF_TAPS(lines, stride) + CVK_AXIS_ALIGN(CVK_AXIS_NLINES(lines) * (size_t)(stride) * 4))
#define CVK_FIR_TVH_LINES 16
typedef struct {
    cvk_view target, source;
    int in_half, out_half;
    int tx0, ty0, tx1, ty1;
    cvk_fir_axis h, v;
    int max_sw, max_sh;
    int nframes, pad_;
    const void *frame_source[8];
    void *frame_target[8];
} cvk_fir2d_params;
#define CVK_FIR2D_TILE_X 32
#define CVK_FIR2D_TILE_Y 16
int cvk_fir_hv_supported(const cvk_fir2d_params *fp);
int cvk_fir_hv(const cvk_fir2d_params *fp, int cus, void *stream);
int cvk_fir_vh_supported(const cvk_fir2d_params *fp);
int cvk_fir_vh(const cvk_fir2d_params *fp, int line0, int cus, void *stream);
int cvk_fir_tvh_supported(const cvk_fir2d_params *fp);
int cvk_fir_tvh_preferred(const cvk_fir2d_params *fp);
int cvk_fir_tvh(const cvk_fir2d_params *fp, int line0, void *stream);
size_t cvk_fir2d_lds_bytes(const cvk_fir2d_params *fp);
int cvk_fir2d(const cvk_fir2d_params *fp, void *stream);

#define CVK_FRAME_BATCH 8
#define CVK_BLUR_MAX_OVER 4
typedef struct {
    int n, pad;
    const void *source[CVK_FRAME_BATCH];
    void *target[CVK_FRAME_BATCH];
    const void *over[CVK_FRAME_BATCH][CVK_BLUR_MAX_OVER];
} cvk_frame_batch;

typedef struct {
    cvk_view target, source;
    int in_half, out_half;
    int tx0, ty0, tx1, ty1;
    int sx0, sy0, sx1, sy1;
    int ntaps;
    int rows_per_wg;
    int step;
    float taps[32];
    int nover;
    int flags;
    const void *over[CVK_BLUR_MAX_OVER];
    cvk_frame_batch batch;
} cvk_blur_params;
#define CVK_BLUR_ONE_COLUMN  1
#define CVK_BLUR_TWO_COLUMNS 2
int cvk_blur_supported(int ntaps, int step);
int cvk_blur(const cvk_blur_params *bp, int cus, void *stream);
int cvk_blur_takes_pairs(const cvk_blur_params *bp);
int cvk_blur_pair_supported(const cvk_blur_params *bp);
int cvk_blur_pair(const cvk_blur_params *bp, int cus, void *stream);

typedef struct {
    cvk_view target, source;
    int in_half, out_half;
    int tx0, ty0, tx1, ty1;
    int sx0, sy0, sx1, sy1;
    int ntaps1, ntaps2;
    int rows_per_wg;
    int flags;
    float taps1[16], taps2[16];
    cvk_frame_batch batch;
} cvk_blur_halve_params;
int cvk_blur_halve_supported(int ntaps1, int ntaps2);
int cvk_blur_halve_pair_supported(const cvk_blur_halve_params *bp);
int cvk_blur_halve_pair(const cvk_blur_halve_params *bp, int cus, void *stream);
int cvk_blur_halve_takes_pairs(const cvk_blur_halve_params *bp);
int cvk_blur_halve(const cvk_blur_halve_params *bp, int cus, void *stream);

typedef struct {
    cvk_view target, source;
    int half;
    int tx0, ty0, tx1, ty1;
    int sx0, sy0, sx1, sy1;
    int ntaps;
    int rows_per_wg;
    float amount, threshold;
    float taps[16];
} cvk_unsharp_params;
int cvk_unsharp_supported(int ntaps);
int cvk_unsharp(const cvk_unsharp_params *up, int cus, void *stream);
int cvk_unsharp_combine(cvk_view out, cvk_view src, cvk_view blurred, cvk_rect r, int half, float amount, float threshold, void *stream);

enum { CVK_DISPLAY_RGBA8 = 0, CVK_DISPLAY_ARGB32_PREMUL = 1 };
int cvk_display(void *dst, cvk_view src, cvk_rect r, const uint8_t *table, int mode, int cus, void *stream);

typedef struct { uint8_t *y, *cb, *cr; int sy, scb, scr; } cvk_dv_planes;
typedef struct { float coeff[16]; int width, center; } cvk_dv_taps;
int cvk_dv_reconstruct(cvk_view frame, cvk_rect cur, const cvk_dv_planes *pl, const cvk_dv_taps *tri, const uint16_t *lut, void *stream);
int cvk_dv_subsample(const cvk_dv_planes *pl, cvk_view frame, cvk_rect w, const cvk_dv_taps *tri, const uint16_t *lut, int encode_in_place, void *stream);

int cvk_mpeg2_subsample(const cvk_dv_planes *pl, cvk_view frame, cvk_rect w, int width, int height, const uint16_t *lut, int cus, void *stream);
int cvk_mpeg2_reconstruct(cvk_view frame, cvk_rect w, const cvk_dv_planes *pl, int width, int height, int progressive, const float mat[9],
                          const uint16_t *lut, int cus, void *stream);

int cvk_field_to_frame(cvk_view out, cvk_view in, cvk_rect w, cvk_rect in_cur, int field, int cus, void *stream);
int cvk_soften_fields(cvk_view out, cvk_view in, cvk_rect w, cvk_rect in_cur, int cus, void *stream);
int cvk_interlace_fields(cvk_view out, cvk_view even, cvk_view odd, cvk_rect w, cvk_rect even_cur, cvk_rect odd_cur, int cus, void *stream);

typedef struct {
    float kpb, kpr, tolerance, inv_soft, inv_spill, spill;
    int soft, fade;
    int matte;
} cvk_key_params;
int cvk_chroma_key(const cvk_key_params *kp, cvk_view out, cvk_view in, cvk_rect w, int half, int cus, void *stream);

#define CVK_MATTE_MAX_LDS (160u << 10)
typedef struct {
    cvk_view out, in;
    cvk_rect w, s;
    int xs;
    int tw, th;
    int r, grow, ntaps;
    int levels, show;
    float black, inv;
    float taps[25];
} cvk_matte_params;
size_t cvk_matte_lds_bytes(int tw, int th, int halo);
int cvk_matte_refine(const cvk_matte_params *mp, int half, void *stream);

typedef struct {
    cvk_view out, in;
    cvk_rect w, s;
    float m[6];
    int bilinear;
    int tw, th;
    int pair_loads;
} cvk_transform_params;
int cvk_transform(const cvk_transform_params *tp, int half, void *stream);

#ifndef CVS_CONTRACT
int cvk_gain_offset_f16_fma(cvk_view out, cvk_view in, cvk_rect r, float gain, float offset, void *stream);
int cvk_mix_fma(const cvk_mix_params *mp, void *stream);
int cvk_color_matrix_fma(cvk_view dst, cvk_view src, cvk_rect r, const float m[9], const uint16_t *pre_lut, const uint16_t *post_lut, int cus, void *stream);
int cvk_chain_color_over_fma(const cvk_chain_job *jobs, int njobs, int uniform_layers, const float *m, const uint16_t *pre_lut, const uint16_t *post_lut, int cus, void *stream);
int cvk_chain_cross_fma(const cvk_chain_job *jobs, int njobs, float wa, float wb, int cus, void *stream);
void cvk_chain_count_reset_fma(void);
int cvk_chain_count_fma(void);
int cvk_fir_gather_fma(const cvk_fir_params *fp, void *stream);
size_t cvk_fir2d_lds_bytes_fma(const cvk_fir2d_params *fp);
int cvk_fir2d_fma(const cvk_fir2d_params *fp, void *stream);
int cvk_fir_vh_supported_fma(const cvk_fir2d_params *fp);
int cvk_fir_vh_fma(const cvk_fir2d_params *fp, int line0, int cus, void *stream);
int cvk_fir_tvh_supported_fma(const cvk_fir2d_params *fp);
int cvk_fir_tvh_preferred_fma(const cvk_fir2d_params *fp);
int cvk_fir_tvh_fma(const cvk_fir2d_params *fp, int line0, void *stream);
int cvk_blur_supported_fma(int ntaps, int step);
int cvk_blur_takes_pairs_fma(const cvk_blur_params *bp);
int cvk_blur_fma(const cvk_blur_params *bp, int cus, void *stream);
int cvk_blur_pair_supported_fma(const cvk_blur_params *bp);
int cvk_blur_pair_fma(const cvk_blur_params *bp, int cus, void *stream);
int cvk_blur_halve_pair_supported_fma(const cvk_blur_halve_params *bp);
int cvk_blur_halve_pair_fma(const cvk_blur_halve_params *bp, int cus, void *stream);
int cvk_blur_halve_supported_fma(int ntaps1, int ntaps2);
int cvk_blur_halve_takes_pairs_fma(const cvk_blur_halve_params *bp);
int cvk_blur_halve_fma(const cvk_blur_halve_params *bp, int cus, void *stream);
int cvk_unsharp_supported_fma(int ntaps);
int cvk_unsharp_fma(const cvk_unsharp_params *up, int cus, void *stream);
int cvk_unsharp_combine_fma(cvk_view out, cvk_view src, cvk_view blurred, cvk_rect r, int half, float amount, float threshold, void *stream);
int cvk_dv_reconstruct_fma(cvk_view frame, cvk_rect cur, const cvk_dv_planes *pl, const cvk_dv_taps *tri, const uint16_t *lut, void *stream);
int cvk_dv_subsample_fma(const cvk_dv_planes *pl, cvk_view frame, cvk_rect w, const cvk_dv_taps *tri, const uint16_t *lut, int encode_in_place, void *stream);
#endif

#ifdef __cplusplus
}
#endif
#endif
```

### canvas_amd/csrc/kernels/lut_common.hpp

```cpp
#pragma once
#include "kernels.h"
#include "pixel_math.hpp"
#include <string.h>

namespace cvs {

constexpr int kWG = 1024;
constexpr int kLutHalfs = 65536;

struct Mat { float m[9]; int plain; int cross; float wa, wb; };

struct MatR { float m0, m1, m2, m3, m4, m5, m6, m7, m8; int plain, cross; float wa, wb; };
#define CVS_MAT_REGS(k) { (k).m[0], (k).m[1], (k).m[2], (k).m[3], (k).m[4], (k).m[5], (k).m[6], (k).m[7], (k).m[8], (k).plain, (k).cross, (k).wa, (k).wb }

typedef uint32_t u32x4 __attribute__((ext_vector_type(4)));
typedef uint32_t u32x2 __attribute__((ext_vector_type(2)));
typedef const u32x4 __attribute__((address_space(1))) *g_cu4;
typedef u32x4 __attribute__((address_space(1))) *g_u4;
typedef const u32x2 __attribute__((address_space(1))) *g_cu2;
typedef u32x2 __attribute__((address_space(1))) *g_u2;
__device__ __forceinline__ uint4 ld4(const void *p, size_t i) { u32x4 v = ((g_cu4)p)[i]; return make_uint4(v.x, v.y, v.z, v.w); }
__device__ __forceinline__ void st4(void *p, size_t i, uint4 v) { u32x4 t = { v.x, v.y, v.z, v.w }; ((g_u4)p)[i] = t; }
__device__ __forceinline__ uint2 ld2(const void *p, size_t i) { u32x2 v = ((g_cu2)p)[i]; return make_uint2(v.x, v.y); }
__device__ __forceinline__ void st2(void *p, size_t i, uint2 v) { u32x2 t = { v.x, v.y }; ((g_u2)p)[i] = t; }

__device__ __forceinline__ void stage_lut(uint16_t *lds, const uint16_t *__restrict__ table) {
    const uint4 *src = reinterpret_cast<const uint4 *>(table);
    uint4 *dst = reinterpret_cast<uint4 *>(lds);
#pragma unroll
    for (int i = 0; i < kLutHalfs * 2 / 16 / kWG; i++) dst[i * kWG + threadIdx.x] = src[i * kWG + threadIdx.x];
    __syncthreads();
}

template <bool IN_LDS>
__device__ __forceinline__ uint32_t gather2(const uint16_t *lut, uint32_t pair) {
    uint32_t lo = lut[pair & 0xFFFFu], hi = lut[pair >> 16];
    return lo | (hi << 16);
}


inline unsigned persistent_grid(int cus, size_t work_items) {
    size_t need = (work_items + kWG - 1) / kWG;
    size_t g = cus > 0 ? (size_t)cus : 256;
    if (need < g) g = need ? need : 1;
    return (unsigned)g;
}

inline Mat make_mat(const float *m) {
    Mat r;
    r.plain = m ? 0 : 1;
    r.cross = 0; r.wa = r.wb = 0.0f;
    for (int i = 0; i < 9; i++) r.m[i] = m ? m[i] : (i % 4 == 0 ? 1.0f : 0.0f);
    return r;
}

}
```

### canvas_amd/stream.py

```python
import ctypes as C

import numpy as np

from . import _lib, synth
from .device import DeviceFrame
from .shard import frames_of_rank

NODE_BYTES_PER_PIXEL = 16 + 16 + 40
BYTES_PER_PIXEL = 16 + 40
OVERLAYS = 3


class GraphStream:

    def __init__(self, width, height, ring=4, matrix=None, pre_lut=_lib.LUT_REC709_TO_LINEAR_SCENE,
                 post_lut=_lib.LUT_NONE, taps=None, overlays=OVERLAYS, first_frame=0, frame_step=1, exact_slots=None, donors=None):
        from . import REC709_RGB_TO_YPBPR
        self.lib = _lib.load()
        self.w, self.h, self.ring, self.overlays = width, height, ring, overlays
        self.full = (0, 0, width - 1, height - 1)
        self.matrix = np.ascontiguousarray(REC709_RGB_TO_YPBPR if matrix is None else matrix, np.float32).reshape(9)
        self.pre_lut, self.post_lut = pre_lut, post_lut
        self.taps = np.ascontiguousarray(synth.gaussian_taps(9, 1.5) if taps is None else taps, np.float32)
        self.slots = []
        nd = 0
        for slot in range(ring):
            exact = exact_slots is None or slot < exact_slots or not donors
            frames = []
            for k in range(overlays + 1):
                d = DeviceFrame(self.full, np.uint16)
                if exact:
                    d.upload(synth.layer_pixels(width, height, k, first_frame + slot * frame_step))
                else:
                    src_frame = donors[(2 * nd) % len(donors)] if k == 0 else donors[(2 * nd + 1) % len(donors)]
                    nd += 1
                    _lib.check(self.lib.cvs_memcpy_d2d(d.ptr, src_frame.ptr, d.nbytes, None), "d2d")
                frames.append(d)
            src, over = frames[0], frames[1:]
            refs = (C.POINTER(_lib.rgba_frame_f16_t) * overlays)(*[C.pointer(o.c) for o in over])
            self.slots.append({"src": src, "over": over, "over_refs": refs, "graded": DeviceFrame(self.full, np.uint16),
                               "out": DeviceFrame(self.full, np.uint16)})
        _lib.check(self.lib.cvs_stream_sync(None), "donor copies")
        self._m = self.matrix.ctypes.data_as(C.POINTER(C.c_float))
        self._t = self.taps.ctypes.data_as(C.POINTER(C.c_float))

    @staticmethod
    def host_inputs(width, height, frame, overlays=OVERLAYS):
        return [synth.layer_frame(width, height, k, frame) for k in range(overlays + 1)]

    def render(self, slot, stream=None):
        s, lib = self.slots[slot % self.ring], self.lib
        _lib.check(lib.cvs_color_matrix_f16_to_dev(s["graded"].ref(), s["src"].ref(), self._m, self.pre_lut, self.post_lut, stream), "colour")
        _lib.check(lib.cvs_blur_over_f16_dev(s["out"].ref(), s["graded"].ref(), self._t, len(self.taps), s["over_refs"],
                                             self.overlays, stream), "blur+over")
        return s["out"]

    def render_batch(self, slots, stream=None):
        lib, n = self.lib, len(slots)
        ss = [self.slots[i % self.ring] for i in slots]
        for s in ss:
            _lib.check(lib.cvs_color_matrix_f16_to_dev(s["graded"].ref(), s["src"].ref(), self._m, self.pre_lut, self.post_lut, stream), "colour")
        key = tuple(i % self.ring for i in slots)
        if getattr(self, "_batch_key", None) != key:
            fp = C.POINTER(_lib.rgba_frame_f16_t)
            self._b_out = (fp * n)(*[C.pointer(s["out"].c) for s in ss])
            self._b_src = (fp * n)(*[C.pointer(s["graded"].c) for s in ss])
            self._b_ov = (fp * (n * self.overlays))(*[C.pointer(o.c) for s in ss for o in s["over"]])
            self._batch_key = key
        _lib.check(lib.cvs_blur_over_f16_batch_dev(self._b_out, self._b_src, self._t, len(self.taps), self._b_ov, self.overlays, n, stream), "blur+over batch")
        return [s["out"] for s in ss]

    def run(self, frames_per_rank, rank=0, world=1, stream=None):
        mine = frames_of_rank(rank, world, frames_per_rank)
        for i, _g in enumerate(mine):
            self.render(i, stream)
        return len(mine)
```

### include/canvas_hip.h

```cpp
#ifndef CANVAS_HIP_H
#define CANVAS_HIP_H

#include <stdint.h>
#include <stddef.h>
#include <stdbool.h>

#if defined(__cplusplus)
extern "C" {
#endif

#define CVS_EXPORT __attribute__((visibility("default")))
#define NS_PER_SEC INT64_C(1000000000)


typedef uint16_t half;
#define HALF_COUNT 65536

typedef struct { int32_t n; uint32_t d; } rational;
typedef struct { int32_t x, y; } v2i;
typedef struct { v2i min, max; } box2i;
typedef struct { float x, y; } v2f;
typedef struct { v2f min, max; } box2f;

typedef struct { half r, g, b, a; } rgba_f16;
typedef struct { uint8_t r, g, b, a; } rgba_u8;
typedef struct { float r, g, b, a; } rgba_f32;

enum { CVS_MAX_COORD = 1 << 30, CVS_RESAMPLE_MAX_COORD = 1 << 23 };
typedef struct { rgba_f16 *data; box2i full_window; box2i current_window; } rgba_frame_f16;
typedef struct { rgba_f32 *data; box2i full_window; box2i current_window; } rgba_frame_f32;

enum { CVS_FORMAT_F16 = 1, CVS_FORMAT_F32 = 2 };
typedef struct {
    void *data;
    int format;
    box2i full_window;
    box2i current_window;
    void *stream;
} rgba_frame_dev;

typedef void (*video_get_frame_func)(void *self, int frame_index, rgba_frame_f16 *frame);
typedef void (*video_get_frame_32_func)(void *self, int frame_index, rgba_frame_f32 *frame);
typedef void (*video_get_frame_dev_func)(void *self, int frame_index, rgba_frame_dev *frame);

#define VIDEO_SOURCE_FLAG_DEVICE 0x1

typedef struct {
    int flags;
    video_get_frame_func get_frame;
    video_get_frame_32_func get_frame_32;
    video_get_frame_dev_func get_frame_dev;
} video_frame_source_funcs;

typedef struct { void *obj; video_frame_source_funcs *funcs; } video_source;

typedef struct { float *coeff; int width; int center; } fir_filter;


static inline void v2i_add(v2i *r, const v2i *a, const v2i *b) { r->x = a->x + b->x; r->y = a->y + b->y; }
static inline void v2i_subtract(v2i *r, const v2i *a, const v2i *b) { r->x = a->x - b->x; r->y = a->y - b->y; }

#if !defined(__cplusplus)
static inline int min(int a, int b) { return a < b ? a : b; }
static inline int max(int a, int b) { return a > b ? a : b; }
static inline int clamp(int v, int lo, int hi) { return min(max(v, lo), hi); }
#endif
static inline float minf(float a, float b) { return a < b ? a : b; }
static inline float maxf(float a, float b) { return a > b ? a : b; }
static inline float clampf(float v, float lo, float hi) { return minf(maxf(v, lo), hi); }

static inline void box2i_set(box2i *b, int x0, int y0, int x1, int y1) { b->min.x = x0; b->min.y = y0; b->max.x = x1; b->max.y = y1; }
static inline void box2i_set_empty(box2i *b) { box2i_set(b, 0, 0, -1, -1); }
static inline bool box2i_is_empty(const box2i *b) { return b->max.x < b->min.x || b->max.y < b->min.y; }
static inline void box2i_intersect(box2i *r, const box2i *a, const box2i *b) {
    int x0 = a->min.x > b->min.x ? a->min.x : b->min.x, y0 = a->min.y > b->min.y ? a->min.y : b->min.y;
    int x1 = a->max.x < b->max.x ? a->max.x : b->max.x, y1 = a->max.y < b->max.y ? a->max.y : b->max.y;
    box2i_set(r, x0, y0, x1, y1);
}
static inline void box2i_union(box2i *r, const box2i *a, const box2i *b) {
    int x0 = a->min.x < b->min.x ? a->min.x : b->min.x, y0 = a->min.y < b->min.y ? a->min.y : b->min.y;
    int x1 = a->max.x > b->max.x ? a->max.x : b->max.x, y1 = a->max.y > b->max.y ? a->max.y : b->max.y;
    box2i_set(r, x0, y0, x1, y1);
}
static inline void box2i_normalize(box2i *b) {
    if (b->min.x > b->max.x) { int32_t t = b->min.x - 1; b->min.x = b->max.x + 1; b->max.x = t; }
    if (b->min.y > b->max.y) { int32_t t = b->min.y - 1; b->min.y = b->max.y + 1; b->max.y = t; }
}
static inline void box2i_get_size(const box2i *b, v2i *r) {
    r->x = b->max.x < b->min.x ? 0 : b->max.x - b->min.x + 1;
    r->y = b->max.y < b->min.y ? 0 : b->max.y - b->min.y + 1;
}
static inline rgba_f16 *video_get_pixel_f16(rgba_frame_f16 *f, int x, int y) {
    return &f->data[(ptrdiff_t)(y - f->full_window.min.y) * (f->full_window.max.x - f->full_window.min.x + 1) + x - f->full_window.min.x];
}
static inline rgba_f32 *video_get_pixel_f32(rgba_frame_f32 *f, int x, int y) {
    return &f->data[(ptrdiff_t)(y - f->full_window.min.y) * (f->full_window.max.x - f->full_window.min.x + 1) + x - f->full_window.min.x];
}


CVS_EXPORT void init_half(void);
CVS_EXPORT extern void (*half_convert_from_float)(half *out, const float *in, int count);
CVS_EXPORT extern void (*half_convert_to_float)(float *out, const half *in, int count);
CVS_EXPORT extern void (*half_convert_from_float_fast)(half *out, const float *in, int count);
CVS_EXPORT extern void (*half_convert_to_float_fast)(float *out, const half *in, int count);
CVS_EXPORT extern void (*half_lookup)(const half *table, half *out, const half *in, int count);

static inline void rgba_f32_to_f16(rgba_f16 *out, const rgba_f32 *in, int count) { half_convert_from_float(&out->r, &in->r, count * 4); }
static inline void rgba_f16_to_f32(rgba_f32 *out, const rgba_f16 *in, int count) { half_convert_to_float(&out->r, &in->r, count * 4); }

CVS_EXPORT int64_t get_frame_time(const rational *frame_rate, int frame);
CVS_EXPORT int get_time_frame(const rational *frame_rate, int64_t time);
CVS_EXPORT int64_t gettime(void);

CVS_EXPORT void video_get_frame_f16(video_source *source, int frame_index, rgba_frame_f16 *frame);
CVS_EXPORT void video_get_frame_f32(video_source *source, int frame_index, rgba_frame_f32 *frame);
CVS_EXPORT void video_get_frame_f16_gl(video_source *source, int frame_index, rgba_frame_f16 *frame);
CVS_EXPORT void video_get_frame_f32_gl(video_source *source, int frame_index, rgba_frame_f32 *frame);
CVS_EXPORT void video_get_frame_dev(video_source *source, int frame_index, rgba_frame_dev *frame);

CVS_EXPORT void video_copy_frame_f16(rgba_frame_f16 *out, rgba_frame_f16 *in);
CVS_EXPORT void video_copy_frame_alpha_f32(rgba_frame_f32 *out, rgba_frame_f32 *in, float alpha);
CVS_EXPORT void video_attenuate_f32(rgba_frame_f32 *frame, float alpha);
CVS_EXPORT void video_mix_cross_f32(rgba_frame_f32 *out, rgba_frame_f32 *a, rgba_frame_f32 *b, float mix_b);
CVS_EXPORT void video_mix_cross_f32_pull(rgba_frame_f32 *out, video_source *a, int frame_a, video_source *b, int frame_b, float mix_b);
CVS_EXPORT void video_mix_over_f32(rgba_frame_f32 *out, rgba_frame_f32 *b, float mix_b);

CVS_EXPORT void video_scale_bilinear_f32(rgba_frame_f32 *target, v2f target_point, rgba_frame_f32 *source, v2f source_point, v2f factors);
CVS_EXPORT void video_scale_bilinear_f32_pull(rgba_frame_f32 *target, v2f target_point, video_source *source, int frame,
                                              box2i *source_rect, v2f source_point, v2f factors);

CVS_EXPORT void video_transfer_rec709_to_linear_scene(half *out, const half *in, size_t count);
CVS_EXPORT void video_transfer_rec709_to_linear_display(half *out, const half *in, size_t count);
CVS_EXPORT void video_transfer_linear_to_rec709(half *out, const half *in, size_t count);
CVS_EXPORT void video_transfer_linear_to_sRGB(half *out, const half *in, size_t count);
CVS_EXPORT const uint8_t *video_get_gamma45_ramp(void);

CVS_EXPORT void video_color_rgb_to_xyz_sdtv(rgba_frame_f16 *frame);
CVS_EXPORT void video_color_xyz_to_srgb(rgba_frame_f16 *frame);

CVS_EXPORT void filter_createTriangle(float sub, float offset, fir_filter *filter);
CVS_EXPORT void filter_createLanczos(float sub, int kernel_size, float offset, fir_filter *filter);
CVS_EXPORT void filter_free(fir_filter *filter);

CVS_EXPORT void video_filter_gain_offset_f16(rgba_frame_f16 *out, rgba_frame_f16 *in, float gain, float offset);

CVS_EXPORT void video_fill_solid_f16(rgba_frame_f16 *frame, const box2i *window, const rgba_f32 *color);
CVS_EXPORT void video_fill_solid_f32(rgba_frame_f32 *frame, const box2i *window, const rgba_f32 *color);

typedef struct workspace_t_tag workspace_t;
typedef struct workspace_item_t_tag workspace_item_t;
CVS_EXPORT workspace_t *workspace_create(void);
CVS_EXPORT int workspace_get_length(workspace_t *workspace);
CVS_EXPORT workspace_item_t *workspace_add_item(workspace_t *self, void *source, int64_t x, int64_t width, int64_t offset, int64_t z, void *tag);
CVS_EXPORT workspace_item_t *workspace_get_item(workspace_t *self, int index);
CVS_EXPORT void workspace_remove_item(workspace_item_t *item);
CVS_EXPORT void workspace_as_video_source(workspace_t *workspace, video_source *source);
CVS_EXPORT void workspace_free(workspace_t *workspace);
CVS_EXPORT void workspace_get_item_pos(workspace_item_t *item, int64_t *x, int64_t *width, int64_t *z);
CVS_EXPORT int64_t workspace_get_item_offset(workspace_item_t *item);
CVS_EXPORT void workspace_set_item_offset(workspace_item_t *item, int64_t offset);
CVS_EXPORT void *workspace_get_item_source(workspace_item_t *item);
CVS_EXPORT void workspace_set_item_source(workspace_item_t *item, void *source);
CVS_EXPORT void *workspace_get_item_tag(workspace_item_t *item);
CVS_EXPORT void workspace_set_item_tag(workspace_item_t *item, void *tag);
CVS_EXPORT void workspace_update_item(workspace_item_t *item, int64_t *x, int64_t *width, int64_t *z, int64_t *offset, void **source, void **tag);


typedef void *cvs_stream_t;

enum { CVS_LUT_NONE = -1, CVS_LUT_REC709_TO_LINEAR_SCENE = 0, CVS_LUT_REC709_TO_LINEAR_DISPLAY = 1,
       CVS_LUT_LINEAR_TO_REC709 = 2, CVS_LUT_LINEAR_TO_SRGB = 3, CVS_LUT_COUNT = 4 };

enum { CVS_ARITH_SEPARATE = 0, CVS_ARITH_CONTRACTED = 1 };
CVS_EXPORT int cvs_set_arithmetic(int mode);
CVS_EXPORT int cvs_get_arithmetic(void);

CVS_EXPORT int cvs_init(int device);
CVS_EXPORT int cvs_device_count(void);
CVS_EXPORT int cvs_current_device(void);

CVS_EXPORT int cvs_context_open(int device);
CVS_EXPORT int cvs_context_count(void);
CVS_EXPORT int cvs_context_device(int ctx);
CVS_EXPORT int cvs_set_context(int ctx);
CVS_EXPORT int cvs_current_context(void);
CVS_EXPORT int cvs_frame_owner(int64_t frame_index, int nowners);
CVS_EXPORT const char *cvs_last_error(void);
CVS_EXPORT void cvs_clear_last_error(void);
enum { CVS_LOG_ERROR = 0, CVS_LOG_WARNING = 1, CVS_LOG_INFO = 2 };
typedef void (*cvs_log_func)(const char *domain, int level, const char *message, void *user_data);
CVS_EXPORT void cvs_set_log_handler(cvs_log_func handler, void *user_data);
CVS_EXPORT const char *cvs_device_name(void);
CVS_EXPORT int cvs_compute_units(void);

CVS_EXPORT void *cvs_malloc(size_t bytes);
CVS_EXPORT void cvs_free(void *dev);
typedef void *cvs_graph_t;
CVS_EXPORT int cvs_graph_begin(cvs_stream_t stream);
CVS_EXPORT cvs_graph_t cvs_graph_end(cvs_stream_t stream);
CVS_EXPORT int cvs_graph_launch(cvs_graph_t graph, cvs_stream_t stream);
CVS_EXPORT void cvs_graph_destroy(cvs_graph_t graph);
CVS_EXPORT int cvs_mem_info(size_t *free_bytes, size_t *total_bytes);
CVS_EXPORT void *cvs_pool_malloc(size_t bytes, cvs_stream_t s);
CVS_EXPORT void cvs_pool_free(void *dev, cvs_stream_t s);
CVS_EXPORT void cvs_pool_trim(void);
CVS_EXPORT void cvs_thread_release(void);
CVS_EXPORT int cvs_memcpy_h2d(void *dev, const void *host, size_t bytes, cvs_stream_t s);
CVS_EXPORT int cvs_memcpy_d2h(void *host, const void *dev, size_t bytes, cvs_stream_t s);
CVS_EXPORT int cvs_memcpy_d2d(void *dst, const void *src, size_t bytes, cvs_stream_t s);
CVS_EXPORT int cvs_memset(void *dev, int value, size_t bytes, cvs_stream_t s);
CVS_EXPORT cvs_stream_t cvs_stream_create(void);
CVS_EXPORT void cvs_stream_destroy(cvs_stream_t s);
CVS_EXPORT int cvs_stream_sync(cvs_stream_t s);
typedef void *cvs_event_t;
CVS_EXPORT cvs_event_t cvs_event_create(void);
CVS_EXPORT void cvs_event_destroy(cvs_event_t e);
CVS_EXPORT int cvs_event_record(cvs_event_t e, cvs_stream_t s);
CVS_EXPORT int cvs_event_sync(cvs_event_t e);
CVS_EXPORT float cvs_event_elapsed_ms(cvs_event_t start, cvs_event_t stop);

CVS_EXPORT const half *cvs_lut_device(int which);
CVS_EXPORT const half *cvs_lut_host(int which);
CVS_EXPORT int cvs_lut_install(int which, const half *table_host);

CVS_EXPORT int cvs_half_to_float_dev(float *out, const half *in, size_t count, cvs_stream_t s);
CVS_EXPORT int cvs_float_to_half_dev(half *out, const float *in, size_t count, cvs_stream_t s);
CVS_EXPORT int cvs_half_to_float_fast_dev(float *out, const half *in, size_t count, cvs_stream_t s);
CVS_EXPORT int cvs_float_to_half_fast_dev(half *out, const float *in, size_t count, cvs_stream_t s);
CVS_EXPORT int cvs_half_lookup_dev(const half *table_dev, half *out, const half *in, size_t count, cvs_stream_t s);

CVS_EXPORT int cvs_frame_f16_to_f32_dev(rgba_frame_f32 *out, const rgba_frame_f16 *in, cvs_stream_t s);
CVS_EXPORT int cvs_frame_f32_to_f16_dev(rgba_frame_f16 *out, const rgba_frame_f32 *in, cvs_stream_t s);
CVS_EXPORT int cvs_copy_frame_f16_dev(rgba_frame_f16 *out, const rgba_frame_f16 *in, cvs_stream_t s);
CVS_EXPORT int cvs_copy_frame_alpha_f32_dev(rgba_frame_f32 *out, const rgba_frame_f32 *in, float alpha, cvs_stream_t s);
CVS_EXPORT int cvs_mix_cross_f32_dev(rgba_frame_f32 *out, const rgba_frame_f32 *a, const rgba_frame_f32 *b, float mix_b, cvs_stream_t s);
CVS_EXPORT int cvs_mix_over_f32_dev(rgba_frame_f32 *out, const rgba_frame_f32 *b, float mix_b, cvs_stream_t s);
CVS_EXPORT int cvs_color_matrix_f16_dev(rgba_frame_f16 *frame, const float m[9], int pre_lut, int post_lut, cvs_stream_t s);
CVS_EXPORT int cvs_color_matrix_f16_to_dev(rgba_frame_f16 *out, const rgba_frame_f16 *in, const float m[9], int pre_lut, int post_lut, cvs_stream_t s);
CVS_EXPORT int cvs_gain_offset_f16_dev(rgba_frame_f16 *out, const rgba_frame_f16 *in, float gain, float offset, cvs_stream_t s);
CVS_EXPORT int cvs_fill_solid_f16_dev(rgba_frame_f16 *frame, const box2i *window, const rgba_f32 *color, cvs_stream_t s);
CVS_EXPORT int cvs_fill_solid_f32_dev(rgba_frame_f32 *frame, const box2i *window, const rgba_f32 *color, cvs_stream_t s);
CVS_EXPORT int cvs_scale_bilinear_f16_dev(rgba_frame_f16 *target, v2f tp, const rgba_frame_f16 *source, v2f sp, v2f fac, cvs_stream_t stream);
CVS_EXPORT int cvs_scale_bilinear_f32_batch_dev(rgba_frame_f32 *const *targets, v2f target_point, const rgba_frame_f32 *const *sources, v2f source_point,
                                                v2f factors, int count, cvs_stream_t stream);
CVS_EXPORT int cvs_scale_bilinear_f16_batch_dev(rgba_frame_f16 *const *targets, v2f target_point, const rgba_frame_f16 *const *sources, v2f source_point,
                                                v2f factors, int count, cvs_stream_t stream);
CVS_EXPORT int cvs_scale_bilinear_f32_dev(rgba_frame_f32 *target, v2f target_point, const rgba_frame_f32 *source, v2f source_point, v2f factors, cvs_stream_t s);
CVS_EXPORT int cvs_fir_blur_f32_dev(rgba_frame_f32 *target, const rgba_frame_f32 *source, const float *taps_host, int ntaps, cvs_stream_t s);
#define CODED_IMAGE_MAX_PLANES 4
typedef struct {
    void *data[CODED_IMAGE_MAX_PLANES];
    int stride[CODED_IMAGE_MAX_PLANES];
    int line_count[CODED_IMAGE_MAX_PLANES];
    void (*free_func)(void *image);
} coded_image;
CVS_EXPORT coded_image *coded_image_alloc(const int *strides, const int *line_counts, int count);
CVS_EXPORT coded_image *coded_image_alloc0(const int *strides, const int *line_counts, int count);
CVS_EXPORT void video_reconstruct_dv(rgba_frame_f16 *frame, coded_image *planar);
CVS_EXPORT coded_image *video_subsample_dv(rgba_frame_f16 *frame);
CVS_EXPORT int cvs_reconstruct_dv_dev(rgba_frame_f16 *frame, const coded_image *planar, cvs_stream_t stream);
CVS_EXPORT int cvs_subsample_dv_dev(coded_image *planar, rgba_frame_f16 *frame, int encode_input_in_place, cvs_stream_t stream);
CVS_EXPORT coded_image *video_subsample_mpeg2(rgba_frame_f16 *frame);
CVS_EXPORT int cvs_subsample_mpeg2_dev(coded_image *planar, const rgba_frame_f16 *frame, int width, int height, cvs_stream_t stream);
enum { CVS_YCC_PROGRESSIVE = 1, CVS_YCC_REC709 = 2 };
CVS_EXPORT int cvs_reconstruct_mpeg2_dev(rgba_frame_f16 *frame, const coded_image *planar, int width, int height, int flags, cvs_stream_t stream);
CVS_EXPORT void video_reconstruct_mpeg2(rgba_frame_f16 *frame, coded_image *planar);

CVS_EXPORT int cvs_pulldown23_frames(int offset, int frame_index, int *first, int *second);
CVS_EXPORT int cvs_weave_fields_f16_dev(rgba_frame_f16 *frame, const rgba_frame_f16 *other, cvs_stream_t stream);

CVS_EXPORT int cvs_field_to_frame_f16_dev(rgba_frame_f16 *out, const rgba_frame_f16 *in, int field, cvs_stream_t stream);
CVS_EXPORT int cvs_soften_fields_f16_dev(rgba_frame_f16 *out, const rgba_frame_f16 *in, cvs_stream_t stream);
CVS_EXPORT int cvs_interlace_fields_f16_dev(rgba_frame_f16 *out, const rgba_frame_f16 *even, const rgba_frame_f16 *odd, cvs_stream_t stream);
CVS_EXPORT int cvs_pulldown23_add_frames(int offset, int frame_index, int *even_source, int *odd_source);

enum { CVS_DISPLAY_RGBA8 = 0, CVS_DISPLAY_ARGB32_PREMUL = 1 };
CVS_EXPORT int cvs_frame_to_bytes_dev(void *dst_dev, const rgba_frame_f16 *frame, int pre_lut, int mode, cvs_stream_t stream);
CVS_EXPORT int video_frame_to_bytes(void *dst_host, const rgba_frame_f16 *host_frame, int pre_lut, int mode);
CVS_EXPORT int cvs_frame_to_rgba8_intent_dev(void *dst_dev, const rgba_frame_f16 *frame, int pre_lut, float rendering_intent, cvs_stream_t stream);
CVS_EXPORT int video_frame_to_rgba8_intent(void *dst_host, const rgba_frame_f16 *host_frame, int pre_lut, float rendering_intent);

CVS_EXPORT int cvs_fir_blur_f16_dev(rgba_frame_f16 *target, const rgba_frame_f16 *source, const float *taps, int ntaps, cvs_stream_t stream);
CVS_EXPORT int cvs_unsharp_mask_f32_dev(rgba_frame_f32 *target, const rgba_frame_f32 *source, const float *taps, int ntaps, float amount, float threshold, cvs_stream_t s);
CVS_EXPORT int cvs_unsharp_mask_f16_dev(rgba_frame_f16 *target, const rgba_frame_f16 *source, const float *taps, int ntaps, float amount, float threshold, cvs_stream_t s);
enum { CVS_KEY_SHOW_MATTE = 1 };
typedef struct cvs_chroma_key {
    float key[3];
    float tolerance;
    float softness;
    float spill;
    float spill_range;
    int   flags;
} cvs_chroma_key;
CVS_EXPORT int cvs_chroma_key_f32_dev(rgba_frame_f32 *target, const rgba_frame_f32 *source, const cvs_chroma_key *key, cvs_stream_t s);
CVS_EXPORT int cvs_chroma_key_f16_dev(rgba_frame_f16 *target, const rgba_frame_f16 *source, const cvs_chroma_key *key, cvs_stream_t s);
enum { CVS_MATTE_SHOW = 1 };
enum { CVS_MATTE_MAX_CHOKE = 16, CVS_MATTE_MAX_TAPS = 25 };
typedef struct cvs_matte {
    float black, white;
    int   choke;
    int   ntaps;
    const float *taps;
    int   flags;
} cvs_matte;
CVS_EXPORT int cvs_matte_refine_f32_dev(rgba_frame_f32 *target, const rgba_frame_f32 *source, const cvs_matte *m, cvs_stream_t s);
CVS_EXPORT int cvs_matte_refine_f16_dev(rgba_frame_f16 *target, const rgba_frame_f16 *source, const cvs_matte *m, cvs_stream_t s);
enum { CVS_TRANSFORM_NEAREST = 0, CVS_TRANSFORM_BILINEAR = 1 };
enum { CVS_TRANSFORM_MAX_COORD = 1 << 23 };
typedef struct cvs_transform {
    float m[6];
    int   filter;
    int   flags;
} cvs_transform;
CVS_EXPORT int cvs_transform_f32_dev(rgba_frame_f32 *target, const rgba_frame_f32 *source, const cvs_transform *t, cvs_stream_t s);
CVS_EXPORT int cvs_transform_f16_dev(rgba_frame_f16 *target, const rgba_frame_f16 *source, const cvs_transform *t, cvs_stream_t s);
CVS_EXPORT int cvs_transform_from_parts(const double anchor[2], const double scale[2], double rotation_degrees, const double position[2], float m[6]);
CVS_EXPORT int cvs_transform_target_window(const cvs_transform *t, const box2i *source_current, const box2i *target_full, box2i *win);
CVS_EXPORT int cvs_transform_source_window(const cvs_transform *t, const box2i *target_window, box2i *need);
CVS_EXPORT int cvs_blur_over_f16_dev(rgba_frame_f16 *out, const rgba_frame_f16 *source, const float *taps, int ntaps,
                                     const rgba_frame_f16 *const *overlays, int noverlays, cvs_stream_t stream);
CVS_EXPORT int cvs_resample_lanczos_f32_dev(rgba_frame_f32 *target, const rgba_frame_f32 *source, float factor_x, float factor_y, int kernel_size, cvs_stream_t s);
CVS_EXPORT int cvs_resample_lanczos_f16_dev(rgba_frame_f16 *target, const rgba_frame_f16 *source, float factor_x, float factor_y, int kernel_size, cvs_stream_t s);
CVS_EXPORT int cvs_blur_lanczos_f16_dev(rgba_frame_f16 *target, const rgba_frame_f16 *source, const float *taps_host, int ntaps,
                                        float factor_x, float factor_y, int kernel_size, cvs_stream_t s);
CVS_EXPORT int cvs_blur_over_f16_batch_dev(rgba_frame_f16 *const *outs, const rgba_frame_f16 *const *sources, const float *taps, int ntaps,
                                           const rgba_frame_f16 *const *overlays, int noverlays, int count, cvs_stream_t stream);
CVS_EXPORT int cvs_blur_lanczos_f16_batch_dev(rgba_frame_f16 *const *targets, const rgba_frame_f16 *const *sources, int count,
                                              const float *taps_host, int ntaps, float fx, float fy, int ksize, cvs_stream_t stream);

enum { CVS_FIR_PATH_AUTO = 0, CVS_FIR_PATH_PASSES = 1 , CVS_FIR_PATH_TILED = 2, CVS_FIR_PATH_TABLES = 4 ,
       CVS_FIR_PATH_HV = 16 ,
       CVS_FIR_PATH_ONE_COLUMN = 32 ,
       CVS_FIR_PATH_TWO_COLUMNS = 64 ,
       CVS_FIR_PATH_STRIPS = 128 ,
       CVS_FIR_PATH_TILES = 256  };
CVS_EXPORT void cvs_fir_path_override(int mode);
enum { CVS_FIR_KERNEL_NONE = 0,
       CVS_FIR_KERNEL_WINDOW = 1,
       CVS_FIR_KERNEL_HALVE = 2,
       CVS_FIR_KERNEL_VH = 4,
       CVS_FIR_KERNEL_TILED = 5,
       CVS_FIR_KERNEL_RETIRED_6 = 6,
       CVS_FIR_KERNEL_TWO_PASS = 7,
       CVS_FIR_KERNEL_PASS = 8,
       CVS_FIR_KERNEL_HV = 9,
       CVS_FIR_KERNEL_WINDOW_PAIR = 10,
       CVS_FIR_KERNEL_HALVE_PAIR = 11,
       CVS_FIR_KERNEL_TILE_VH = 12,
       CVS_FIR_KERNEL_UNSHARP = 13 };
CVS_EXPORT int cvs_fir_last_kernel(void);
CVS_EXPORT int cvs_fir_fell_through_count(void);

#define CVS_CHAIN_MAX_LAYERS 8
typedef struct {
    rgba_frame_f16 *out;
    const rgba_frame_f16 *layers[CVS_CHAIN_MAX_LAYERS];
    int nlayers;
} cvs_chain_job;
CVS_EXPORT int cvs_chain_color_over_f16_dev(const cvs_chain_job *jobs, int njobs, const float m[9],
                                            int pre_lut, int post_lut, cvs_stream_t s);
CVS_EXPORT int cvs_chain_last_was_fused(void);
CVS_EXPORT int cvs_scale_last_was_fused(void);
CVS_EXPORT int cvs_chain_last_launch_count(void);
CVS_EXPORT int cvs_mix_cross_f16_dev(rgba_frame_f16 *out, const rgba_frame_f16 *a, const rgba_frame_f16 *b, float mix_b, cvs_stream_t stream);

#if defined(__cplusplus)
}
#endif
#endif
```

Baseline: 259,600.

## Fuse source colour grade into the blur+over pair kernel

Adds a blur kernel that applies the colour matrix and optional LUT to each source row as it loads it. The stream renderer now sets a pending grade and calls blur+over on the raw source instead of first writing a graded intermediate frame. This removes one full-frame write and read of HBM traffic per frame, at the cost of doing the grade inside the blur loop. It also adds LDS use for the LUT and introduces thread-local state that passes the grade between calls. BYTES_PER_PIXEL in the metric accounting is lowered to match the reduced traffic.

```diff
diff --git a/canvas_amd/_lib.py b/canvas_amd/_lib.py
--- a/canvas_amd/_lib.py
+++ b/canvas_amd/_lib.py
@@ -214,6 +214,7 @@
     "cvs_resample_lanczos_f16_dev": (C.c_int, [_F16, _F16, C.c_float, C.c_float, C.c_int, _vp]),
     "cvs_blur_lanczos_f16_dev": (C.c_int, [_F16, _F16, _f32p, C.c_int, C.c_float, C.c_float, C.c_int, _vp]),
     "cvs_blur_over_f16_batch_dev": (C.c_int, [P(_F16), P(_F16), _f32p, C.c_int, P(_F16), C.c_int, C.c_int, _vp]),
+    "cvs_blur_source_grade": (C.c_int, [_f32p, C.c_int, C.c_int]),
     "cvs_scale_bilinear_f16_batch_dev": (C.c_int, [P(_F16), v2f, P(_F16), v2f, v2f, C.c_int, _vp]),
     "cvs_scale_bilinear_f32_batch_dev": (C.c_int, [P(_F32), v2f, P(_F32), v2f, v2f, C.c_int, _vp]),
     "cvs_blur_lanczos_f16_batch_dev": (C.c_int, [P(_F16), P(_F16), C.c_int, _f32p, C.c_int, C.c_float, C.c_float, C.c_int, _vp]),
diff --git a/canvas_amd/csrc/host/scale.c b/canvas_amd/csrc/host/scale.c
--- a/canvas_amd/csrc/host/scale.c
+++ b/canvas_amd/csrc/host/scale.c
@@ -468,8 +468,10 @@
     return 0;
 }
 
-static int blur_fused(const any_frame *t, const any_frame *src, const box2i *win, const float *taps, int ntaps,
-                      const void *const *over, int nover, const cvk_frame_batch *batch, hipStream_t s) {
+typedef struct { float m[9]; int pre_lut, post_lut; } source_grade;
+
+static int blur_fused_graded(const any_frame *t, const any_frame *src, const box2i *win, const float *taps, int ntaps,
+                             const void *const *over, int nover, const cvk_frame_batch *batch, const source_grade *grade, hipStream_t s) {
     const box2i *sw = &src->cur;
     if (blur_has_fast_kernel(taps, ntaps)) {
         cvk_blur_params bp;
@@ -488,16 +490,31 @@
             bp.batch = *batch;
         }
         bp.flags = blur_column_pins();
+        if (grade) {
+            if (bp.flags & CVK_BLUR_ONE_COLUMN) return 1;
+            const half *pre = cvs_lut_dev_or_null(grade->pre_lut), *post = cvs_lut_dev_or_null(grade->post_lut);
+            if ((grade->pre_lut != CVS_LUT_NONE && !pre) || (grade->post_lut != CVS_LUT_NONE && !post)) return -1;
+            if (!CVK(cvk_blur_grade_pair_supported)(&bp, grade->m, pre, post)) return 1;
+            int rc = CVK(cvk_blur_grade_pair)(&bp, grade->m, pre, post, cvs_cus(), s);
+            if (rc != 0) { cvs_set_error("blur launch failed: %s", hipGetErrorString((hipError_t)rc)); return -1; }
+            t_fir_kernel = CVS_FIR_KERNEL_WINDOW_PAIR;
+            return 0;
+        }
         int rc = CVK(cvk_blur)(&bp, cvs_cus(), s);
         if (rc != 0) { cvs_set_error("blur launch failed: %s", hipGetErrorString((hipError_t)rc)); return -1; }
         t_fir_kernel = CVK(cvk_blur_takes_pairs)(&bp) ? CVS_FIR_KERNEL_WINDOW_PAIR : CVS_FIR_KERNEL_WINDOW;
         return 0;
     }
-    if (nover > 0 || batch) return 1;
+    if (nover > 0 || batch || grade) return 1;
     cvs_fir_table h, v;
     if (cvs_fir_table_blur(taps, ntaps, win->min.x, win->max.x, sw->min.x, sw->max.x, CVK_FIR2D_TILE_X, &h) != 0) return -1;
     if (cvs_fir_table_blur(taps, ntaps, win->min.y, win->max.y, sw->min.y, sw->max.y, CVK_FIR2D_TILE_Y, &v) != 0) { cvs_fir_table_release(&h, s); return -1; }
     return fir_pair_launch(t, src, win, &h, &v, s);
+}
+
+static int blur_fused(const any_frame *t, const any_frame *src, const box2i *win, const float *taps, int ntaps,
+                      const void *const *over, int nover, const cvk_frame_batch *batch, hipStream_t s) {
+    return blur_fused_graded(t, src, win, taps, ntaps, over, nover, batch, NULL, s);
 }
 
 static int lanczos_fused(const any_frame *t, const any_frame *src, float fx, float fy, int ksize, hipStream_t s) {
@@ -605,15 +622,59 @@
     return unsharp_mask(target, source, taps, ntaps, amount, threshold, 1, s, "cvs_unsharp_mask_f16_dev");
 }
 
+static _Thread_local struct { int set; source_grade g; } t_source_grade;
+
+CVS_EXPORT int cvs_blur_source_grade(const float *m, int pre_lut, int post_lut) {
+    t_source_grade.set = 0;
+    if (!m) return 0;
+    memcpy(t_source_grade.g.m, m, sizeof t_source_grade.g.m);
+    t_source_grade.g.pre_lut = pre_lut; t_source_grade.g.post_lut = post_lut;
+    t_source_grade.set = 1;
+    return 0;
+}
+
+static const source_grade *take_source_grade(source_grade *g) {
+    if (!t_source_grade.set) return NULL;
+    *g = t_source_grade.g;
+    t_source_grade.set = 0;
+    return g;
+}
+
+static int blur_over_one(rgba_frame_f16 *out, const rgba_frame_f16 *source, const float *taps, int ntaps,
+                         const rgba_frame_f16 *const *overlays, int noverlays, const source_grade *grade, cvs_stream_t stream);
+
+static int blur_over_graded_frame(rgba_frame_f16 *out, const rgba_frame_f16 *source, const float *taps, int ntaps,
+                                  const rgba_frame_f16 *const *overlays, int noverlays, const source_grade *grade, cvs_stream_t stream) {
+    hipStream_t s = cvs_pick_stream(stream);
+    rgba_frame_f16 graded = { NULL, source->full_window, source->full_window };
+    graded.data = cvs_pool_malloc(cvs_box_pixels(&source->full_window) * sizeof(rgba_f16), s);
+    if (!graded.data) { box2i_set_empty(&out->current_window); return -1; }
+    int rc = cvs_color_matrix_f16_to_dev(&graded, source, grade->m, grade->pre_lut, grade->post_lut, stream);
+    if (rc == 0) rc = blur_over_one(out, &graded, taps, ntaps, overlays, noverlays, NULL, stream);
+    else box2i_set_empty(&out->current_window);
+    cvs_pool_free(graded.data, s);
+    return rc;
+}
+
 CVS_EXPORT int cvs_blur_over_f16_dev(rgba_frame_f16 *out, const rgba_frame_f16 *source, const float *taps, int ntaps,
                                      const rgba_frame_f16 *const *overlays, int noverlays, cvs_stream_t stream) {
+    source_grade g;
+    const source_grade *grade = take_source_grade(&g);
+    return blur_over_one(out, source, taps, ntaps, overlays, noverlays, grade, stream);
+}
+
+static int blur_over_one(rgba_frame_f16 *out, const rgba_frame_f16 *source, const float *taps, int ntaps,
+                         const rgba_frame_f16 *const *overlays, int noverlays, const source_grade *grade, cvs_stream_t stream) {
     if (cvs_enter() != 0) { box2i_set_empty(&out->current_window); return -1; }
     CVS_REQUIRE_INSIDE(source, out, "cvs_blur_over_f16_dev");
     CVS_REQUIRE_COORDS(source, 1, out, "cvs_blur_over_f16_dev", "source");
     CVS_REQUIRE_COORDS(out, 0, out, "cvs_blur_over_f16_dev", "out");
     for (int l = 0; l < noverlays && overlays; l++) CVS_REQUIRE_COORDS(overlays[l], 1, out, "cvs_blur_over_f16_dev", "an overlay");
     if (ntaps < 1 || !taps || noverlays < 0 || (noverlays > 0 && !overlays)) { cvs_set_error("blur+over: bad arguments"); box2i_set_empty(&out->current_window); return -1; }
-    if (noverlays == 0) return cvs_fir_blur_f16_dev(out, source, taps, ntaps, stream);
+    if (noverlays == 0) {
+        if (grade && !box2i_is_empty(&source->current_window)) return blur_over_graded_frame(out, source, taps, ntaps, overlays, 0, grade, stream);
+        return cvs_fir_blur_f16_dev(out, source, taps, ntaps, stream);
+    }
     hipStream_t s = cvs_pick_stream(stream);
     const box2i *full = &out->full_window;
     if (box2i_is_empty(full)) { box2i_set_empty(&out->current_window); return 0; }
@@ -627,9 +688,10 @@
         bufs[l] = overlays[l]->data;
     }
     int rc = 1;
-    if (whole && noverlays > 0) rc = blur_fused(&o, &src, &win, taps, ntaps, bufs, noverlays, NULL, s);
+    if (whole && noverlays > 0) rc = blur_fused_graded(&o, &src, &win, taps, ntaps, bufs, noverlays, NULL, grade, s);
     if (rc == 0) { out->current_window = *full; return 0; }
     if (rc < 0) { box2i_set_empty(&out->current_window); return rc; }
+    if (grade && !box2i_is_empty(&source->current_window)) return blur_over_graded_frame(out, source, taps, ntaps, overlays, noverlays, grade, stream);
 
     rgba_frame_f32 acc = { cvs_pool_malloc(cvs_box_pixels(full) * sizeof(rgba_f32), s), *full, *full };
     rgba_frame_f32 tmp = { noverlays > 0 ? cvs_pool_malloc(cvs_box_pixels(full) * sizeof(rgba_f32), s) : NULL, *full, *full };
@@ -711,6 +773,8 @@
 CVS_EXPORT int cvs_blur_over_f16_batch_dev(rgba_frame_f16 *const *outs, const rgba_frame_f16 *const *sources, const float *taps, int ntaps,
                                            const rgba_frame_f16 *const *overlays, int noverlays, int count, cvs_stream_t stream) {
     const char *what = "cvs_blur_over_f16_batch_dev";
+    source_grade g;
+    const source_grade *grade = take_source_grade(&g);
     if (count <= 0) return 0;
     if (ntaps < 1 || !taps || noverlays < 0 || (noverlays > 0 && !overlays)) { cvs_set_error("%s: bad arguments", what); return -1; }
     for (int i = 0; i < count; i++)
@@ -737,12 +801,12 @@
         cvk_frame_batch b;
         if (!batch_group(&b, outs, sources, 1, done, n, bytes, bytes, overlays, noverlays)) break;
         const any_frame t = { b.target[0], *full, *full, 1 }, src = { (void *)b.source[0], sources[done]->full_window, sources[done]->current_window, 1 };
-        rc = blur_fused(&t, &src, full, taps, ntaps, b.over[0], noverlays, &b, s);
+        rc = blur_fused_graded(&t, &src, full, taps, ntaps, b.over[0], noverlays, &b, grade, s);
         if (rc == 1) { rc = 0; break; }
         if (rc == 0) { for (int i = 0; i < n; i++) outs[done + i]->current_window = *full; done += n; }
     }
     for (; rc == 0 && done < count; done++)
-        rc = cvs_blur_over_f16_dev(outs[done], sources[done], taps, ntaps, noverlays ? overlays + (size_t)done * noverlays : NULL, noverlays, stream);
+        rc = blur_over_one(outs[done], sources[done], taps, ntaps, noverlays ? overlays + (size_t)done * noverlays : NULL, noverlays, grade, stream);
     if (rc != 0) batch_empty_from(outs, done, count, 1);
     return rc;
 }
diff --git a/canvas_amd/csrc/kernels/blur_grade_pair_ops.hip b/canvas_amd/csrc/kernels/blur_grade_pair_ops.hip
--- /dev/null
+++ b/canvas_amd/csrc/kernels/blur_grade_pair_ops.hip
@@ -0,0 +1,230 @@
+#include <cstdlib>
+#include "pair_common.hpp"
+
+namespace {
+
+using namespace pairsweep;
+using cvs::kLutHalfs;
+
+constexpr int waves_for(int nt, int nov) { return (nt <= 7 || (nt == 9 && nov <= 3)) ? 12 : 8; }
+
+__device__ __forceinline__ void wave_lds_order() {
+    __builtin_amdgcn_fence(__ATOMIC_RELEASE, "wavefront");
+    __builtin_amdgcn_wave_barrier();
+    __builtin_amdgcn_fence(__ATOMIC_ACQUIRE, "wavefront");
+}
+
+template <int NT, int NOV, bool PRE, bool POST, int kWaves = waves_for(NT, NOV)>
+__global__ __launch_bounds__(kWaves * 64) void k_blur_grade_pair(cvk_blur_params bp, cvs::Mat kmat, const uint16_t *__restrict__ table,
+                                                            int strips, int segs, int nitems) {
+    constexpr int W = 64, C = NT / 2, D = C & 1, OUTW = 2 * W - 2 * C - 2 * D, PITCH = W + 8;
+    static_assert(NT & 1 && NT >= 3 && NT <= 13, "odd tap counts up to 13");
+    static_assert(NOV >= 1 && NOV <= CVK_BLUR_MAX_OVER, "layer count");
+    static_assert(!(PRE && POST), "one table in LDS");
+    constexpr bool TABLE = PRE || POST;
+    __shared__ uint16_t lut[TABLE ? kLutHalfs : 1];
+    __shared__ float4 rowbuf[kWaves][2][PITCH];
+    const cvs::MatR mat = CVS_MAT_REGS(kmat);
+    const int wave = __builtin_amdgcn_readfirstlane((int)(threadIdx.x >> 6)), lane = (int)(threadIdx.x & 63);
+    float4 (*buf)[PITCH] = rowbuf[wave];
+
+    if (lane < PITCH - W) {
+#pragma unroll
+        for (int ph = 0; ph < 2; ph++) buf[ph][W + lane] = make_float4(0.f, 0.f, 0.f, 0.f);
+    }
+    if constexpr (TABLE) cvs::stage_lut_any(lut, table);
+
+    float w[NT];
+#pragma unroll
+    for (int k = 0; k < NT; k++) w[k] = bp.taps[k];
+
+    typedef const cvk_blur_params __attribute__((address_space(4))) *kargs_t;
+    const kargs_t ka = (kargs_t)__builtin_amdgcn_kernarg_segment_ptr();
+    const size_t srow = (size_t)bp.source.pitch * 8, trow = (size_t)bp.target.pitch * 8;
+    const uint32_t swin = (uint32_t)(bp.sx1 - bp.sx0 + 1) * 8u, trect = (uint32_t)(bp.tx1 - bp.tx0 + 1) * 8u;
+    const ptrdiff_t trect0 = (ptrdiff_t)(bp.tx0 - bp.target.fx0) * 8;
+
+    for (int item = (int)blockIdx.x * kWaves + wave; item < nitems; item += (int)gridDim.x * kWaves) {
+        const int strip = item % strips, rest = item / strips, seg = rest % segs, z = rest / segs;
+        const int xo = bp.tx0 + strip * OUTW;
+        const int sfirst = xo - C - D;
+        const int tcol = xo + 2 * lane;
+        const int ta = bp.ty0 + seg * bp.rows_per_wg;
+        const int tb = min(ta + bp.rows_per_wg - 1, bp.ty1);
+        const int ys0 = ta - C;
+        const int steps = (tb - ta) + NT;
+
+        const void *src_data = bp.batch.n ? ka->batch.source[z] : bp.source.data;
+        void *dst_data = bp.batch.n ? ka->batch.target[z] : bp.target.data;
+        const void *over_data[NOV];
+#pragma unroll
+        for (int l = 0; l < NOV; l++) over_data[l] = bp.batch.n ? ka->batch.over[z][l] : bp.over[l];
+
+        const uint32_t soff = (uint32_t)((sfirst + 2 * lane - bp.sx0) * 8);
+        const uint32_t toff = 2 * lane < OUTW ? (uint32_t)((tcol - bp.tx0) * 8) : 0x80000000u;
+        const bool in_cols = soff < swin;
+        const char *swin0 = reinterpret_cast<const char *>(src_data) + (ptrdiff_t)(bp.sx0 - bp.source.fx0) * 8;
+
+        Px ring[NT][2];
+#pragma unroll
+        for (int k = 0; k < NT; k++) ring[k][0].rg = ring[k][0].ba = ring[k][1].rg = ring[k][1].ba = f32x2{ 0.0f, 0.0f };
+
+        auto row_live = [&](int ys, bool wanted) { return wanted && ys >= bp.sy0 && ys <= bp.sy1; };
+        auto fetch_row = [&](int ys, bool wanted) {
+            return load_pair(row_rsrc(swin0, (size_t)((ptrdiff_t)(ys - bp.source.fy0) * (ptrdiff_t)srow), row_live(ys, wanted) ? swin : 0u), soff);
+        };
+        auto grade_row = [&](u32x4 raw, int ys, bool wanted) {
+            const u32x4 g = cvs::color_pair_codes<PRE, POST>(raw, mat, lut, nullptr);
+            return (in_cols && row_live(ys, wanted)) ? g : u32x4{ 0u, 0u, 0u, 0u };
+        };
+        struct Layers { u32x4 v[NOV]; };
+        auto fetch_layers = [&](int i) {
+            Layers r;
+            const bool emits = i >= NT - 1 && i < steps;
+            const size_t o = (size_t)((ptrdiff_t)(ta + i - (NT - 1) - bp.target.fy0) * (ptrdiff_t)trow + trect0);
+#pragma unroll
+            for (int l = 0; l < NOV; l++) r.v[l] = load_pair(row_rsrc(over_data[l], o, emits ? trect : 0u), toff);
+            return r;
+        };
+        u32x4 g = fetch_row(ys0, true);
+        u32x4 cur = fetch_row(ys0 + 1, steps > 1);
+        Layers ov_cur = fetch_layers(0);
+        g = grade_row(g, ys0, true);
+        wave_lds_order();
+        buf[0][lane] = widen_px(g.x, g.y);
+        buf[1][lane] = widen_px(g.z, g.w);
+        g = grade_row(cur, ys0 + 1, steps > 1);
+        cur = fetch_row(ys0 + 2, steps > 2);
+
+        for (int i0 = 0; i0 < steps; i0 += NT) {
+            auto step = [&](auto jc) -> bool {
+                constexpr int j = decltype(jc)::value;
+                const int i = i0 + j;
+                if (i >= steps) return false;
+                const bool emits = i >= NT - 1;
+                const int t = ta + (i - (NT - 1));
+                const u32x4 far = fetch_row(ys0 + i + 3, i + 3 < steps);
+                const Layers ov_nxt = fetch_layers(i + 1);
+                wave_lds_order();
+                float4 v[NT + 1];
+#pragma unroll
+                for (int c = 0; c <= NT; c++) v[c] = buf[(c + D) & 1][lane + ((c + D) >> 1)];
+                wave_lds_order();
+                buf[0][lane] = widen_px(g.x, g.y);
+                buf[1][lane] = widen_px(g.z, g.w);
+                g = grade_row(cur, ys0 + i + 2, i + 2 < steps);
+                cur = far;
+                f32x2 rg0, ba0, rg1, ba1;
+#pragma unroll
+                for (int k = 0; k < NT; k++) {
+                    if constexpr (cvs::kContract) {
+                        if (k == 0) { rg0 = f32x2{ v[0].x, v[0].y } * w[0]; ba0 = f32x2{ v[0].z, v[0].w } * w[0]; rg1 = f32x2{ v[1].x, v[1].y } * w[0]; ba1 = f32x2{ v[1].z, v[1].w } * w[0]; }
+                        else {
+                            rg0 = cvs::madd(f32x2{ v[k].x, v[k].y }, w[k], rg0); ba0 = cvs::madd(f32x2{ v[k].z, v[k].w }, w[k], ba0);
+                            rg1 = cvs::madd(f32x2{ v[k + 1].x, v[k + 1].y }, w[k], rg1); ba1 = cvs::madd(f32x2{ v[k + 1].z, v[k + 1].w }, w[k], ba1);
+                        }
+                    } else {
+                    const f32x2 p0 = f32x2{ v[k].x, v[k].y } * w[k], q0 = f32x2{ v[k].z, v[k].w } * w[k];
+                    const f32x2 p1 = f32x2{ v[k + 1].x, v[k + 1].y } * w[k], q1 = f32x2{ v[k + 1].z, v[k + 1].w } * w[k];
+                    if (k == 0) { rg0 = p0; ba0 = q0; rg1 = p1; ba1 = q1; }
+                    else { rg0 = rg0 + p0; ba0 = ba0 + q0; rg1 = rg1 + p1; ba1 = ba1 + q1; }
+                    }
+                }
+                ring[j][0].rg = rg0; ring[j][0].ba = ba0;
+                ring[j][1].rg = rg1; ring[j][1].ba = ba1;
+                if (emits) {
+                    f32x2 org0, oba0, org1, oba1;
+#pragma unroll
+                    for (int k = 0; k < NT; k++) {
+                        const Px &a = ring[(j + 1 + k) % NT][0], &b = ring[(j + 1 + k) % NT][1];
+                        if constexpr (cvs::kContract) {
+                            if (k == 0) { org0 = a.rg * w[0]; oba0 = a.ba * w[0]; org1 = b.rg * w[0]; oba1 = b.ba * w[0]; }
+                            else { org0 = cvs::madd(a.rg, w[k], org0); oba0 = cvs::madd(a.ba, w[k], oba0); org1 = cvs::madd(b.rg, w[k], org1); oba1 = cvs::madd(b.ba, w[k], oba1); }
+                        } else {
+                        const f32x2 p0 = a.rg * w[k], q0 = a.ba * w[k], p1 = b.rg * w[k], q1 = b.ba * w[k];
+                        if (k == 0) { org0 = p0; oba0 = q0; org1 = p1; oba1 = q1; }
+                        else { org0 = org0 + p0; oba0 = oba0 + q0; org1 = org1 + p1; oba1 = oba1 + q1; }
+                        }
+                    }
+                    cvs::px32x2 acc;
+                    acc.r = f32x2{ org0.x, org1.x }; acc.g = f32x2{ org0.y, org1.y };
+                    acc.b = f32x2{ oba0.x, oba1.x }; acc.a = f32x2{ oba0.y, oba1.y };
+#pragma unroll
+                    for (int l = 0; l < NOV; l++) acc = cvs::over_pair_uniform(acc, ov_cur.v[l]);
+                    const u32x4 codes = cvs::narrow_pair_lean(acc);
+                    __builtin_amdgcn_raw_buffer_store_b128(codes, row_rsrc(dst_data, (size_t)((ptrdiff_t)(t - bp.target.fy0) * (ptrdiff_t)trow + trect0), trect), (int)toff, 0, 0);
+                }
+                ov_cur = ov_nxt;
+                return true;
+            };
+            each_slot(step, std::make_integer_sequence<int, NT>{});
+        }
+    }
+}
+
+template <int NT, int NOV, bool PRE, bool POST>
+int launch(cvk_blur_params bp, const cvs::Mat &mat, const uint16_t *table, int cus, hipStream_t s) {
+    constexpr int C = NT / 2, D = C & 1, OUTW = 2 * 64 - 2 * C - 2 * D, kWaves = waves_for(NT, NOV);
+    const int cols = bp.tx1 - bp.tx0 + 1, rows = bp.ty1 - bp.ty0 + 1;
+    const int strips = (cols + OUTW - 1) / OUTW;
+    const int ncu = cus > 0 ? cus : 256;
+    const int nframes = bp.batch.n > 0 ? bp.batch.n : 1;
+    if (bp.rows_per_wg <= 0) {
+        int want = (kWaves * ncu) / (strips * nframes);
+        if (want < 1) want = 1;
+        int r = (rows + want - 1) / want;
+        if (r < NT - 1) r = NT - 1;
+        if (r > rows) r = rows;
+        bp.rows_per_wg = r;
+    }
+    const int segs = (rows + bp.rows_per_wg - 1) / bp.rows_per_wg;
+    const long long items = (long long)strips * segs * nframes;
+    if (items > 0x7fffff00LL) return (int)hipErrorInvalidValue;
+    long long wgs = (items + kWaves - 1) / kWaves;
+    if (wgs > ncu) wgs = ncu;
+    hipLaunchKernelGGL((k_blur_grade_pair<NT, NOV, PRE, POST>), dim3((unsigned)wgs), dim3(kWaves * 64), 0, s, bp, mat, table, strips, segs, (int)items);
+    return (int)hipGetLastError();
+}
+
+template <int NT, int NOV>
+int pick_table(const cvk_blur_params *bp, const cvs::Mat &mat, const uint16_t *pre, const uint16_t *post, int cus, hipStream_t s) {
+    if (pre) return launch<NT, NOV, true, false>(*bp, mat, pre, cus, s);
+    if (post) return launch<NT, NOV, false, true>(*bp, mat, post, cus, s);
+    return launch<NT, NOV, false, false>(*bp, mat, nullptr, cus, s);
+}
+
+template <int NT>
+int pick_layers(const cvk_blur_params *bp, const cvs::Mat &mat, const uint16_t *pre, const uint16_t *post, int cus, hipStream_t s) {
+    switch (bp->nover) {
+    case 1: return pick_table<NT, 1>(bp, mat, pre, post, cus, s);
+    case 2: return pick_table<NT, 2>(bp, mat, pre, post, cus, s);
+    case 3: return pick_table<NT, 3>(bp, mat, pre, post, cus, s);
+    case 4: return pick_table<NT, 4>(bp, mat, pre, post, cus, s);
+    }
+    return (int)hipErrorInvalidValue;
+}
+
+}
+
+extern "C" int cvk_blur_grade_pair_supported(const cvk_blur_params *bp, const float *m, const uint16_t *pre, const uint16_t *post) {
+    return m && !(pre && post) && bp->nover >= 1 && cvk_blur_pair_supported(bp);
+}
+
+extern "C" int cvk_blur_grade_pair(const cvk_blur_params *bp_in, const float *m, const uint16_t *pre, const uint16_t *post, int cus, void *stream) {
+    if (bp_in->tx1 < bp_in->tx0 || bp_in->ty1 < bp_in->ty0) return 0;
+    if (!cvk_blur_grade_pair_supported(bp_in, m, pre, post)) return (int)hipErrorInvalidValue;
+    cvk_blur_params bp = *bp_in;
+    bp.step = 1;
+    bp.flags = 0;
+    const cvs::Mat mat = cvs::make_mat(m);
+    hipStream_t s = (hipStream_t)stream;
+    switch (bp.ntaps) {
+    case 3: return pick_layers<3>(&bp, mat, pre, post, cus, s);
+    case 5: return pick_layers<5>(&bp, mat, pre, post, cus, s);
+    case 7: return pick_layers<7>(&bp, mat, pre, post, cus, s);
+    case 9: return pick_layers<9>(&bp, mat, pre, post, cus, s);
+    case 11: return pick_layers<11>(&bp, mat, pre, post, cus, s);
+    case 13: return pick_layers<13>(&bp, mat, pre, post, cus, s);
+    }
+    return (int)hipErrorInvalidValue;
+}
diff --git a/canvas_amd/csrc/kernels/chain_kernel.hpp b/canvas_amd/csrc/kernels/chain_kernel.hpp
--- a/canvas_amd/csrc/kernels/chain_kernel.hpp
+++ b/canvas_amd/csrc/kernels/chain_kernel.hpp
@@ -60,22 +60,6 @@
     else asm volatile("s_waitcnt vmcnt(0)" : "+v"(r[0]), "+v"(r[1]), "+v"(r[2]), "+v"(r[3]), "+v"(r[4]), "+v"(r[5]), "+v"(r[6]), "+v"(r[7]) : : "memory");
 }
 
-__device__ __forceinline__ void stage_lut_any(uint16_t *lds, const uint16_t *__restrict__ table) {
-    const uint4 *src = reinterpret_cast<const uint4 *>(table);
-    uint4 *dst = reinterpret_cast<uint4 *>(lds);
-    constexpr int kWords = kLutHalfs * 2 / 16;
-    if (kWords % blockDim.x == 0) {
-        const int slices = kWords / (int)blockDim.x, rot = (int)(blockIdx.x >> 3);
-        for (int it = 0; it < slices; it++) {
-            const int i = ((it + rot) % slices) * (int)blockDim.x + (int)threadIdx.x;
-            dst[i] = src[i];
-        }
-    } else {
-        for (int i = threadIdx.x; i < kWords; i += blockDim.x) dst[i] = src[i];
-    }
-    __syncthreads();
-}
-
 enum { DIAG_NONE = 0, DIAG_MEMORY_ONLY = 1, DIAG_COMPUTE_ONLY = 2 };
 
 template <int NL>
diff --git a/canvas_amd/csrc/kernels/kernels.h b/canvas_amd/csrc/kernels/kernels.h
--- a/canvas_amd/csrc/kernels/kernels.h
+++ b/canvas_amd/csrc/kernels/kernels.h
@@ -32,6 +32,8 @@
 #define cvk_blur                     cvk_blur_fma
 #define cvk_blur_pair_supported      cvk_blur_pair_supported_fma
 #define cvk_blur_pair                cvk_blur_pair_fma
+#define cvk_blur_grade_pair_supported cvk_blur_grade_pair_supported_fma
+#define cvk_blur_grade_pair          cvk_blur_grade_pair_fma
 #define cvk_blur_halve_pair_supported cvk_blur_halve_pair_supported_fma
 #define cvk_blur_halve_pair          cvk_blur_halve_pair_fma
 #define cvk_blur_halve_supported     cvk_blur_halve_supported_fma
@@ -190,6 +192,8 @@
 int cvk_blur_takes_pairs(const cvk_blur_params *bp);
 int cvk_blur_pair_supported(const cvk_blur_params *bp);
 int cvk_blur_pair(const cvk_blur_params *bp, int cus, void *stream);
+int cvk_blur_grade_pair_supported(const cvk_blur_params *bp, const float *m, const uint16_t *pre_lut, const uint16_t *post_lut);
+int cvk_blur_grade_pair(const cvk_blur_params *bp, const float *m, const uint16_t *pre_lut, const uint16_t *post_lut, int cus, void *stream);
 
 typedef struct {
     cvk_view target, source;
@@ -290,6 +294,8 @@
 int cvk_blur_fma(const cvk_blur_params *bp, int cus, void *stream);
 int cvk_blur_pair_supported_fma(const cvk_blur_params *bp);
 int cvk_blur_pair_fma(const cvk_blur_params *bp, int cus, void *stream);
+int cvk_blur_grade_pair_supported_fma(const cvk_blur_params *bp, const float *m, const uint16_t *pre_lut, const uint16_t *post_lut);
+int cvk_blur_grade_pair_fma(const cvk_blur_params *bp, const float *m, const uint16_t *pre_lut, const uint16_t *post_lut, int cus, void *stream);
 int cvk_blur_halve_pair_supported_fma(const cvk_blur_halve_params *bp);
 int cvk_blur_halve_pair_fma(const cvk_blur_halve_params *bp, int cus, void *stream);
 int cvk_blur_halve_supported_fma(int ntaps1, int ntaps2);
diff --git a/canvas_amd/csrc/kernels/lut_common.hpp b/canvas_amd/csrc/kernels/lut_common.hpp
--- a/canvas_amd/csrc/kernels/lut_common.hpp
+++ b/canvas_amd/csrc/kernels/lut_common.hpp
@@ -32,6 +32,22 @@
     __syncthreads();
 }
 
+__device__ __forceinline__ void stage_lut_any(uint16_t *lds, const uint16_t *__restrict__ table) {
+    const uint4 *src = reinterpret_cast<const uint4 *>(table);
+    uint4 *dst = reinterpret_cast<uint4 *>(lds);
+    constexpr int kWords = kLutHalfs * 2 / 16;
+    if (kWords % blockDim.x == 0) {
+        const int slices = kWords / (int)blockDim.x, rot = (int)(blockIdx.x >> 3);
+        for (int it = 0; it < slices; it++) {
+            const int i = ((it + rot) % slices) * (int)blockDim.x + (int)threadIdx.x;
+            dst[i] = src[i];
+        }
+    } else {
+        for (int i = threadIdx.x; i < kWords; i += blockDim.x) dst[i] = src[i];
+    }
+    __syncthreads();
+}
+
 template <bool IN_LDS>
 __device__ __forceinline__ uint32_t gather2(const uint16_t *lut, uint32_t pair) {
     uint32_t lo = lut[pair & 0xFFFFu], hi = lut[pair >> 16];
diff --git a/canvas_amd/stream.py b/canvas_amd/stream.py
--- a/canvas_amd/stream.py
+++ b/canvas_amd/stream.py
@@ -7,7 +7,7 @@
 from .shard import frames_of_rank
 
 NODE_BYTES_PER_PIXEL = 16 + 16 + 40
-BYTES_PER_PIXEL = 16 + 40
+BYTES_PER_PIXEL = 40
 OVERLAYS = 3
 
 
@@ -38,8 +38,7 @@
                 frames.append(d)
             src, over = frames[0], frames[1:]
             refs = (C.POINTER(_lib.rgba_frame_f16_t) * overlays)(*[C.pointer(o.c) for o in over])
-            self.slots.append({"src": src, "over": over, "over_refs": refs, "graded": DeviceFrame(self.full, np.uint16),
-                               "out": DeviceFrame(self.full, np.uint16)})
+            self.slots.append({"src": src, "over": over, "over_refs": refs, "out": DeviceFrame(self.full, np.uint16)})
         _lib.check(self.lib.cvs_stream_sync(None), "donor copies")
         self._m = self.matrix.ctypes.data_as(C.POINTER(C.c_float))
         self._t = self.taps.ctypes.data_as(C.POINTER(C.c_float))
@@ -50,23 +49,22 @@
 
     def render(self, slot, stream=None):
         s, lib = self.slots[slot % self.ring], self.lib
-        _lib.check(lib.cvs_color_matrix_f16_to_dev(s["graded"].ref(), s["src"].ref(), self._m, self.pre_lut, self.post_lut, stream), "colour")
-        _lib.check(lib.cvs_blur_over_f16_dev(s["out"].ref(), s["graded"].ref(), self._t, len(self.taps), s["over_refs"],
+        _lib.check(lib.cvs_blur_source_grade(self._m, self.pre_lut, self.post_lut), "source grade")
+        _lib.check(lib.cvs_blur_over_f16_dev(s["out"].ref(), s["src"].ref(), self._t, len(self.taps), s["over_refs"],
                                              self.overlays, stream), "blur+over")
         return s["out"]
 
     def render_batch(self, slots, stream=None):
         lib, n = self.lib, len(slots)
         ss = [self.slots[i % self.ring] for i in slots]
-        for s in ss:
-            _lib.check(lib.cvs_color_matrix_f16_to_dev(s["graded"].ref(), s["src"].ref(), self._m, self.pre_lut, self.post_lut, stream), "colour")
         key = tuple(i % self.ring for i in slots)
         if getattr(self, "_batch_key", None) != key:
             fp = C.POINTER(_lib.rgba_frame_f16_t)
             self._b_out = (fp * n)(*[C.pointer(s["out"].c) for s in ss])
-            self._b_src = (fp * n)(*[C.pointer(s["graded"].c) for s in ss])
+            self._b_src = (fp * n)(*[C.pointer(s["src"].c) for s in ss])
             self._b_ov = (fp * (n * self.overlays))(*[C.pointer(o.c) for s in ss for o in s["over"]])
             self._batch_key = key
+        _lib.check(lib.cvs_blur_source_grade(self._m, self.pre_lut, self.post_lut), "source grade")
         _lib.check(lib.cvs_blur_over_f16_batch_dev(self._b_out, self._b_src, self._t, len(self.taps), self._b_ov, self.overlays, n, stream), "blur+over batch")
         return [s["out"] for s in ss]
 
diff --git a/include/canvas_hip.h b/include/canvas_hip.h
--- a/include/canvas_hip.h
+++ b/include/canvas_hip.h
@@ -319,6 +319,7 @@
 CVS_EXPORT int cvs_transform_source_window(const cvs_transform *t, const box2i *target_window, box2i *need);
 CVS_EXPORT int cvs_blur_over_f16_dev(rgba_frame_f16 *out, const rgba_frame_f16 *source, const float *taps, int ntaps,
                                      const rgba_frame_f16 *const *overlays, int noverlays, cvs_stream_t stream);
+CVS_EXPORT int cvs_blur_source_grade(const float *m , int pre_lut, int post_lut);
 CVS_EXPORT int cvs_resample_lanczos_f32_dev(rgba_frame_f32 *target, const rgba_frame_f32 *source, float factor_x, float factor_y, int kernel_size, cvs_stream_t s);
 CVS_EXPORT int cvs_resample_lanczos_f16_dev(rgba_frame_f16 *target, const rgba_frame_f16 *source, float factor_x, float factor_y, int kernel_size, cvs_stream_t s);
 CVS_EXPORT int cvs_blur_lanczos_f16_dev(rgba_frame_f16 *target, const rgba_frame_f16 *source, const float *taps_host, int ntaps,
```

Result: no change. 259,500 (-0.0%).
